# mauruszach/multimodal_diffusion

Measured on AMD Instinct MI355X. Metric: denoising steps/sec @256x256 multimodal-cond batch=32, higher is better.
Workload: dtype f32 via 3xbf16 split operands (6-term products, f32 accumulate; fp32-level error); 1 GPU; C3: 256x256 audio->video CFG denoising step (cond+null MMDiT d512 L8 H8 + noise head + DDIM), 384+37 tokens, batch 32 per GPU, DDIM 50 steps, guidance 3.5; global_batch=32, sampler_steps=50, parallelism=dp1, launch=eager, matmul=bf16x3, attn=default, cfg_halves=two HIP streams

## Files before the change

### multimodal_diffusion_amd/csrc/avd_common.h

```cpp
#pragma once
#include <hip/hip_runtime.h>
#include <stdint.h>
#include <stdio.h>
#include <stdarg.h>
#include <atomic>

#include "../../include/avdiff_hip.h"

namespace avd {

int set_error(int code, const char* fmt, ...);

#define AVD_REQUIRE(cond, code, ...)                       \
    do {                                                   \
        if (!(cond)) return avd::set_error((code), __VA_ARGS__); \
    } while (0)

#define AVD_CHECK_LAUNCH(name)                                                          \
    do {                                                                                \
        hipError_t e__ = hipGetLastError();                                             \
        if (e__ != hipSuccess)                                                          \
            return avd::set_error(AVD_ELAUNCH, "%s: %s", (name), hipGetErrorString(e__)); \
    } while (0)

struct LdsAttr {
    std::atomic<uint64_t> done{0};
    int ensure(const void* kern, int lds_bytes, const char* what);
};

static inline bool aligned16(const void* p) { return (reinterpret_cast<uintptr_t>(p) & 15u) == 0; }

typedef float f32x4 __attribute__((ext_vector_type(4)));
typedef float f32x16 __attribute__((ext_vector_type(16)));

constexpr int kWave = 64;

__device__ __forceinline__ int mfma32_row(int r, int hi) { return (r & 3) + 8 * (r >> 2) + 4 * hi; }

__device__ __forceinline__ float gelu_erf(float x) {
    const float z = x * 0.70710678118654752440f;
    const float a = fabsf(z);
    const float t = __builtin_amdgcn_rcpf(fmaf(0.3275911f, a, 1.0f));
    float p = fmaf(1.061405429f, t, -1.453152027f);
    p = fmaf(p, t, 1.421413741f);
    p = fmaf(p, t, -0.284496736f);
    p = fmaf(p, t, 0.254829592f);
    p *= t;
    const float e = __builtin_amdgcn_exp2f(-a * a * 1.4426950408889634f);
    const float er = copysignf(fmaf(-p, e, 1.0f), z);
    return 0.5f * x * (1.0f + er);
}
__device__ __forceinline__ float silu(float x) { return x / (1.0f + expf(-x)); }

template <int ACT>
__device__ __forceinline__ float apply_act(float x) {
    if constexpr (ACT == AVD_ACT_GELU) return gelu_erf(x);
    else if constexpr (ACT == AVD_ACT_SILU) return silu(x);
    else return x;
}

__device__ __forceinline__ float wave_sum(float v) {
#pragma unroll
    for (int o = 32; o > 0; o >>= 1) v += __shfl_xor(v, o, 64);
    return v;
}

struct RowMap {
    int64_t ld;
    int64_t seg;
    int64_t stride;
    __host__ __device__ __forceinline__ int64_t off(int64_t r) const {
        return seg > 0 ? (r / seg) * stride + (r % seg) * ld : r * ld;
    }
};

struct RowSegs {
    int64_t m0;
    int tok[2], samples[2];
    static RowSegs uniform(int samples, int tok) { return RowSegs{(int64_t)samples * tok, {tok, tok}, {samples, 0}}; }
    __host__ __device__ __forceinline__ int64_t rows() const { return m0 + (int64_t)samples[1] * tok[1]; }
    __host__ __device__ __forceinline__ int n_samples() const { return samples[0] + samples[1]; }
    __host__ __device__ __forceinline__ void locate(int64_t m, int& sample, int& token) const {
        const bool s1 = m >= m0;
        const unsigned r = (unsigned)(s1 ? m - m0 : m), t = (unsigned)(s1 ? tok[1] : tok[0]);
        const unsigned b = r / t;
        sample = (int)b + (s1 ? samples[0] : 0);
        token = (int)(r - b * t);
    }
    __host__ __device__ __forceinline__ int64_t row(int sample, int token) const {
        return sample < samples[0] ? (int64_t)sample * tok[0] + token : m0 + (int64_t)(sample - samples[0]) * tok[1] + token;
    }
};

struct TubeGather {
    int T, H, W, t, h, w, Ht, Wt, Nt;
    int64_t per;
    __host__ __device__ __forceinline__ int64_t row_off(int64_t row) const {
        const int64_t b = row / Nt;
        const int n = (int)(row - b * Nt);
        const int nx = n % Wt, ny = (n / Wt) % Ht, nt = n / (Wt * Ht);
        return b * per + ((int64_t)(nt * t) * H + ny * h) * W + nx * w;
    }
    __host__ __device__ __forceinline__ int64_t k_off(int k) const {
        const int dx = k % w, dy = (k / w) % h, dt = (k / (w * h)) % t, c = k / (w * h * t);
        return (((int64_t)c * T + dt) * H + dy) * W + dx;
    }
};

typedef __bf16 bf16x8 __attribute__((ext_vector_type(8)));
typedef unsigned int u32x4 __attribute__((ext_vector_type(4)));

constexpr int S3_CHUNK = 128 * 96;
constexpr int S3_PLANE = 128 * 32;

typedef __bf16 bf16x2 __attribute__((ext_vector_type(2)));
typedef float f32x2 __attribute__((ext_vector_type(2)));

__device__ __forceinline__ unsigned int pk_bf16(float a, float b) {
    const f32x2 v = {a, b};
    return __builtin_bit_cast(unsigned int, __builtin_convertvector(v, bf16x2));
}
__device__ __forceinline__ float bf16_lo(unsigned int p) { return __uint_as_float(p << 16); }
__device__ __forceinline__ float bf16_hi(unsigned int p) { return __uint_as_float(p & 0xffff0000u); }

template <bool RANGE_CHECK = true>
__device__ __forceinline__ void split8(const float* v, u32x4& H, u32x4& Mi, u32x4& Lo) {
#pragma clang fp contract(off)
    bool edge = false;
    if constexpr (RANGE_CHECK) {
        float amax = fabsf(v[0]);
#pragma unroll
        for (int e = 1; e < 8; ++e) amax = fmaxf(amax, fabsf(v[e]));
        edge = __any(amax > 3.3895313892515355e38f);
    }
#pragma unroll
    for (int e = 0; e < 4; ++e) {
        const float a = v[2 * e], b = v[2 * e + 1];
        unsigned int h = pk_bf16(a, b);
        float ra = a - bf16_lo(h), rb = b - bf16_hi(h);
        if (edge) {
            if ((h & 0x7fffu) == 0x7f80u) {
                if (fabsf(a) < __builtin_inff()) { h = (h & 0xffff8000u) | 0x7f7fu; ra = a - bf16_lo(h); } else ra = 0.f;
            }
            if ((h & 0x7fff0000u) == 0x7f800000u) {
                if (fabsf(b) < __builtin_inff()) { h = (h & 0x8000ffffu) | 0x7f7f0000u; rb = b - bf16_hi(h); } else rb = 0.f;
            }
        }
        const unsigned int m = pk_bf16(ra, rb);
        const float sa = ra - bf16_lo(m), sb = rb - bf16_hi(m);
        H[e] = h;
        Mi[e] = m;
        Lo[e] = pk_bf16(sa, sb);
    }
}

template <bool RANGE_CHECK = true>
__device__ __forceinline__ void store_split8(unsigned char* img, int64_t r, int k, int K, const float* v) {
    u32x4 H, Mi, Lo;
    split8<RANGE_CHECK>(v, H, Mi, Lo);
    const int rr = (int)(r & 127), half = (k >> 3) & 1;
    unsigned char* dst = img + ((r >> 7) * (K >> 4) + (k >> 4)) * (int64_t)S3_CHUNK + rr * 32 + ((half ^ ((rr >> 4) & 1)) << 4);
    *reinterpret_cast<u32x4*>(dst) = H;
    *reinterpret_cast<u32x4*>(dst + S3_PLANE) = Mi;
    *reinterpret_cast<u32x4*>(dst + 2 * S3_PLANE) = Lo;
}

typedef _Float16 f16x8 __attribute__((ext_vector_type(8)));
typedef _Float16 f16x2 __attribute__((ext_vector_type(2)));

__device__ __forceinline__ unsigned int pk_f16(float a, float b) {
    const f32x2 v = {a, b};
    return __builtin_bit_cast(unsigned int, __builtin_convertvector(v, f16x2));
}
__device__ __forceinline__ f32x2 unpk_f16(unsigned int p) { return __builtin_convertvector(__builtin_bit_cast(f16x2, p), f32x2); }

__device__ __forceinline__ void split8_h2(const float* v, float s, u32x4& H, u32x4& L) {
#pragma unroll
    for (int e = 0; e < 4; ++e) {
        const float a = v[2 * e] * s, b = v[2 * e + 1] * s;
        const unsigned int h = pk_f16(a, b);
        const f32x2 u = unpk_f16(h);
        H[e] = h;
        L[e] = pk_f16(a - u[0], b - u[1]);
    }
}
__device__ __forceinline__ void store_split8_h2(unsigned char* img, int64_t r, int k, int K, const float* v, float s) {
    u32x4 H, L;
    split8_h2(v, s, H, L);
    const int rr = (int)(r & 127), half = (k >> 3) & 1;
    unsigned char* dst = img + ((r >> 7) * (K >> 4) + (k >> 4)) * (int64_t)S3_CHUNK + rr * 32 + ((half ^ ((rr >> 4) & 1)) << 4);
    *reinterpret_cast<u32x4*>(dst) = H;
    *reinterpret_cast<u32x4*>(dst + S3_PLANE) = L;
}

template <bool F16>
__device__ __forceinline__ f32x16 mma16(bf16x8 a, bf16x8 b, f32x16 c) {
    if constexpr (F16)
        return __builtin_amdgcn_mfma_f32_32x32x16_f16(__builtin_bit_cast(f16x8, a), __builtin_bit_cast(f16x8, b), c, 0, 0, 0);
    else
        return __builtin_amdgcn_mfma_f32_32x32x16_bf16(a, b, c, 0, 0, 0);
}
__host__ __device__ constexpr int s3_planes(int terms) { return terms == 1 ? 1 : terms == 3 ? 2 : 3; }

constexpr int QKV3_ROWB = 384;
__host__ __device__ __forceinline__ int qkv3_npad(int n) { return (n + 63) / 64 * 64; }
__host__ __device__ __forceinline__ int qkv3_swizzle(int part, int n) {
    return part == 0 ? 0 : part == 1 ? (n >> 1) & 7 : (((n >> 1) & 1) << 2) | (((n >> 2) & 1) << 1);
}

extern bool g_prof_on;
void prof_mark(int tag, double work, hipStream_t st, bool begin);
int prof_tag_id(const char* fmt, ...);
struct ProfScope {
    int tag; hipStream_t st; bool on;
    ProfScope(int t, double work, hipStream_t s) : tag(t), st(s), on(g_prof_on) { if (on) prof_mark(tag, work, st, true); }
    ~ProfScope() { if (on) prof_mark(tag, 0.0, st, false); }
};

int gemm_f32(const float* A, RowMap am, const float* W, const float* bias, const float* R, RowMap rm,
             float* C, RowMap cm, int64_t M, int N, int K, int act, hipStream_t st);
int gemm_f32_tube(const float* z, const TubeGather& tg, const float* W, const float* bias, float* C, RowMap cm, int64_t M, int N, int K,
                  hipStream_t st);

extern int g_gemm_stages;
extern int g_gemm_force_tile;
bool gemm_f32_fold_supported(int N, int K);
int gemm_f32_fold(const float* A, RowMap am, const float* W, const float* bias, const float* R, RowMap rm, float* C, RowMap cm,
                  int64_t M, int N, int K, int act, const float* ss_in, int ss_in_cols, float sqrt_d, float eps, float* ss_out,
                  hipStream_t st);
int rowss_f32(const float* x, float* ss, int64_t rows, int d, hipStream_t st);
constexpr int kGemmSplitKMax = 4;
extern int g_gemm_splitk;
int gemm_f32_splitk_slices(int64_t M, int N, int K);
int64_t gemm_f32_splitk_ws_max_floats(int64_t M, int N, int K);
int gemm_f32_splitk(const float* A, RowMap am, const float* W, const float* bias, const float* R, RowMap rm, float* C, RowMap cm, int64_t M,
                    int N, int K, int ns, float* part, float* ss_out, hipStream_t st);

int attn_f32(const float* qkv, float* out, int B, int N, int H, int Dh, float scale, int n_query, const unsigned char* key_padding_mask,
             hipStream_t st);
int rmsnorm_f32(const float* x, RowMap xm, const float* scale, float* y, RowMap ym, int64_t rows, int d, float eps,
                hipStream_t st);
int layernorm_act_f32(const float* x, const float* gamma, const float* beta, float* y, int64_t rows, int d, float eps,
                      int act, hipStream_t st);
int weight_bounds_f32(const float* x, int64_t rows, int d, float* out2, hipStream_t st);

int64_t split3_bytes(int64_t rows, int K);
int split3_f32(const float* x, int64_t ld, void* out, int64_t rows, int K, hipStream_t st, float h2_scale = 0.f);
int split3_rows_f32(const float* x, RowMap xm, void* out, int64_t rows, int K, hipStream_t st, float h2_scale = 0.f, float* ss = nullptr);
int rmsnorm_split3_f32(const float* x, const float* scale, void* out, int64_t rows, int d, float eps, hipStream_t st, float h2_scale = 0.f);
int layernorm_act_split3_f32(const float* x, const float* gamma, const float* beta, void* out, int64_t rows, int d, float eps, int act,
                             hipStream_t st, float h2_scale = 0.f);
bool gemm_bf16x3_supported(int64_t M, int N, int K);
int attn_f32_split3(const float* qkv, void* out3, int B, int N, int H, int Dh, float scale, int n_query, hipStream_t st);
extern int g_s3_stagger;
extern int g_mlp_fused;
bool mlp_bf16x3_supported(int d, int hidden, int terms);
int mlp_bf16x3(const void* X3, const void* W1n3, const float* b1, const void* W23, const float* b2, const float* ss_in, float eps,
               const float* R, float* C, void* C3, float* ss_out, int64_t M, int d, int hidden, hipStream_t st);
extern int g_attn_m16;
extern int g_attn_pipe;
extern int g_s3_m16;
extern int g_s3_w128;
extern int g_s3_rt4;
extern int g_s3_deep4;
extern int g_s3_rt;
extern int g_vae_lat;
extern int g_vae_fold;
extern int g_codec_mfma;
extern int g_cfg_rows;
extern int g_s3_sn, g_s3_super4, g_s3_super8;
extern int g_s3_tile;
extern thread_local bool t_s3_two_streams;
int gemm_bf16x3_qkv3(const void* A3, const void* W3, const float* bias, void* img, const RowSegs& seg, int heads, int K, float qscale,
                     int terms, hipStream_t st, float ab_scale = 1.f, float c_scale = 1.f, const float* ss_in = nullptr, float eps = 0.f,
                     int64_t plan_rows = 0);
int64_t qkv3_bytes(int B, int N, int H);
int64_t attn_fp8_ws_bytes(int B, int N, int H);
int attn_fp8(const void* qkv3, void* ws, int64_t ws_bytes, float* out, void* out3, int B, int N, int H, int n_query, hipStream_t st,
             int img_terms = 6, float img_scale = 1.f, float out_scale = 1.f);
int attn_bf16x3(const void* qkv3, float* out, void* out3, int B, int N, int H, int n_query, int terms, hipStream_t st,
                float img_scale = 1.f, float out_scale = 1.f, int out_tokens = 0, const RowSegs* out_rows = nullptr);
int gemm_bf16x3(const void* A3, const void* W3, const float* bias, const float* R, float* C, void* C3, int64_t M, int N, int K,
                int act, int terms, hipStream_t st, float ab_scale = 1.f, float c_scale = 1.f, const float* ss_in = nullptr, float eps = 0.f,
                float* ss_out = nullptr, const float* gamma = nullptr, int r_seg = 0, const RowSegs* r_map = nullptr, int64_t plan_rows = 0);
bool gemm_bf16x3_resmap_supported(int terms);
bool gemm_bf16x3_rownorm_supported(int N, int terms);
extern int g_s3_splitk;
int gemm_bf16x3_splitk_slices(int64_t M, int N, int K, int terms);
int64_t gemm_bf16x3_splitk_ws_floats(int64_t M, int N, int ns);
constexpr int kS3SplitKMax = 4;
int64_t gemm_bf16x3_splitk_ws_max_floats(int64_t M, int N, int K);
int gemm_bf16x3_splitk(const void* A3, const void* W3, const float* bias, const float* R, float* C, void* C3, float* ss, int64_t M, int N,
                       int K, int terms, int ns, float* part, hipStream_t st);

}
```

### multimodal_diffusion_amd/csrc/composite.hip

```cpp
#include "avd_common.h"

#include <limits.h>
#include <stdlib.h>

#include <string.h>
#include <map>
#include <mutex>
#include <string>
#include <utility>
#include <vector>

namespace avd {

static thread_local char g_err[512] = "";

int set_error(int code, const char* fmt, ...) {
    va_list ap;
    va_start(ap, fmt);
    vsnprintf(g_err, sizeof(g_err), fmt, ap);
    va_end(ap);
    return code;
}

int LdsAttr::ensure(const void* kern, int lds_bytes, const char* what) {
    int dev = 0;
    hipError_t e = hipGetDevice(&dev);
    if (e != hipSuccess) return set_error(AVD_ELAUNCH, "%s: hipGetDevice: %s", what, hipGetErrorString(e));
    const uint64_t bit = dev < 64 ? (uint64_t)1 << dev : 0;
    if (bit && (done.load(std::memory_order_acquire) & bit)) return AVD_OK;
    e = hipFuncSetAttribute(kern, hipFuncAttributeMaxDynamicSharedMemorySize, lds_bytes);
    if (e != hipSuccess) return set_error(AVD_ELAUNCH, "%s: hipFuncSetAttribute: %s", what, hipGetErrorString(e));
    done.fetch_or(bit, std::memory_order_release);
    return AVD_OK;
}

bool g_prof_on = false;
namespace {
struct ProfRec { hipEvent_t a, b; int tag; double work; };
std::vector<ProfRec> g_recs;
std::vector<hipEvent_t> g_pool;
std::vector<std::string> g_tags;
hipEvent_t take_event() {
    if (!g_pool.empty()) { hipEvent_t e = g_pool.back(); g_pool.pop_back(); return e; }
    hipEvent_t e; (void)hipEventCreate(&e); return e;
}
}
int prof_tag_id(const char* fmt, ...) {
    char buf[160];
    va_list ap;
    va_start(ap, fmt);
    vsnprintf(buf, sizeof(buf), fmt, ap);
    va_end(ap);
    for (size_t i = 0; i < g_tags.size(); ++i)
        if (g_tags[i] == buf) return (int)i;
    g_tags.emplace_back(buf);
    return (int)g_tags.size() - 1;
}
void prof_mark(int tag, double work, hipStream_t st, bool begin) {
    if (begin) {
        ProfRec r{take_event(), take_event(), tag, work};
        (void)hipEventRecord(r.a, st);
        g_recs.push_back(r);
    } else if (!g_recs.empty()) {
        (void)hipEventRecord(g_recs.back().b, st);
    }
}

int temb_f32(const int64_t* t, const float* freqs, float* out, int B, int dim, float max_period, hipStream_t st);
int tube_patch_f32(const float* z, float* tok, int B, int C, int T, int H, int W, int t, int h, int w, hipStream_t st);
int audio_tokens_f32(const float* z, float* tok, int B, int Ca, int F, int len, int stride, hipStream_t st);
int assemble_f32(float* X2, const float* temb, const float* Xp, int B, int N, int d, int tdim, int Nt, int Np,
                 int target_first, hipStream_t st);
int assemble_rows_f32(float* X2, const int64_t* t_now, const float* freqs, const float* Xp, float* ss, int B, int N, int d, int tdim,
                      int Nt, int Np, int target_first, float max_period, hipStream_t st, const RowSegs* short_null = nullptr, int slots = 0,
                      int slot_tok = 0);
int qkv3_replicate(void* img, int img_samples, int H, int n_keys, int first_sample, int n_samples, int src, hipStream_t st);
int cfg_unpatch_ddim_f32(const float* eps2, const float* z, const int64_t* t_now, const int64_t* t_prev,
                         const float* abar, int T_train, float guidance, float eta, const float* noise, float* z_out,
                         int B, int C, int T, int H, int W, int t, int h, int w, hipStream_t st, const avd_noise_key* key = nullptr,
                         const int64_t* t_last = nullptr, float* x0_hist = nullptr, const avd_latent_guide* guide = nullptr,
                         const avd_cfg_control* ctl = nullptr, int canvas_hop = 0, int guide_hop = 0, int slots = 0,
                         const avd_apg_control* apg = nullptr, const avd_slot_key* skey = nullptr,
                         const avd_clip_guide* cguide = nullptr, const avd_slot_cfg* scfg = nullptr);
int cfg_untoken_ddim_audio_f32(const float* eps2, const float* z, const int64_t* t_now, const int64_t* t_prev,
                               const float* abar, int T_train, float guidance, float eta, const float* noise,
                               float* z_out, int B, int Ca, int F, int len, int stride, hipStream_t st,
                               const avd_noise_key* key = nullptr, const int64_t* t_last = nullptr, float* x0_hist = nullptr,
                               const avd_latent_guide* guide = nullptr, const avd_cfg_control* ctl = nullptr, int canvas_hop = 0, int guide_hop = 0,
                               int slots = 0, const avd_apg_control* apg = nullptr, const avd_slot_key* skey = nullptr,
                               const avd_clip_guide* cguide = nullptr, const avd_slot_cfg* scfg = nullptr);
int assemble_cond_f32(float* X1, const float* temb, const float* Xp, int B, int N, int d, int tdim, int Nt, int Np, int target_first,
                      hipStream_t st);
int assemble_rows_cond_f32(float* X1, const int64_t* t_now, const float* freqs, const float* Xp, float* ss, int B, int N, int d,
                           int tdim, int Nt, int Np, int target_first, float max_period, hipStream_t st);
int eps_unpatch_ddim_f32(const float* eps1, const float* z, const int64_t* t_now, const int64_t* t_prev, const float* abar, int T_train,
                         float eta, const float* noise, float* z_out, int B, int C, int T, int H, int W, int t, int h, int w,
                         hipStream_t st, const avd_noise_key* key, const int64_t* t_last, float* x0_hist, const avd_latent_guide* guide,
                         int canvas_hop = 0, int guide_hop = 0);
int eps_untoken_ddim_audio_f32(const float* eps1, const float* z, const int64_t* t_now, const int64_t* t_prev, const float* abar,
                               int T_train, float eta, const float* noise, float* z_out, int B, int Ca, int F, int len, int stride,
                               hipStream_t st, const avd_noise_key* key, const int64_t* t_last, float* x0_hist,
                               const avd_latent_guide* guide, int canvas_hop = 0, int guide_hop = 0);
int check_canvas_key(const avd_noise_key* key, int N, int64_t outer, int L, int hop, int64_t inner);
int check_slot_key(const avd_slot_key* key, int B, int64_t outer, int slot_len, int64_t inner);
int check_clip_guide(const avd_clip_guide* g, int B, int64_t outer, int L, int slots, int slot_len, int64_t inner, const float* out,
                     const float* x0_hist);
int check_canvas_guide(const avd_latent_guide* g, int N, int64_t outer, int L, int hop, int64_t inner, const float* out,
                       const float* x0_hist);
int check_latent_guide(const avd_latent_guide* g, int B, int64_t per, const float* out, const float* x0_hist);
int check_cfg_control(const avd_cfg_control* ctl, int B, int64_t per, const float* out, const float* x0_hist);
int check_apg_control(const avd_apg_control* apg, const avd_cfg_control* ctl, int B, int64_t per, const float* z, const float* out,
                      const float* x0_hist, const void* eps, int64_t eps_bytes);
int check_slot_cfg(const avd_slot_cfg* cfg, int B, int S, int64_t per_slot, int64_t per, const float* z, const float* out,
                   const float* x0_hist, const void* eps, int64_t eps_bytes);
bool overlaps(const float* a, const float* b, int64_t n);

static inline int64_t align_up(int64_t x) { return (x + 255) & ~(int64_t)255; }

struct Carver {
    char* base;
    int64_t used, cap;
    bool ok = true;
    float* take(int64_t floats) {
        float* p = reinterpret_cast<float*>(base + used);
        used += align_up(floats * (int64_t)sizeof(float));
        if (used > cap) ok = false;
        return p;
    }
};

constexpr int64_t kSplitMinRows = 6144;
constexpr int64_t kSplitMinRowsM16 = 2048;
static int g_s3_min_rows = -1;
static int g_no_fold = 0;
static int64_t split_min_rows(int terms = 3) {
    if (g_s3_min_rows >= 0) return g_s3_min_rows;
    return (terms == 0 || terms == 6) && g_s3_m16 ? kSplitMinRowsM16 : kSplitMinRows;
}
static bool core_split_capable(const avd_core_weights* w, int64_t M) {
    if (w->norm_kind != 0) return false;
    if (!gemm_bf16x3_supported(M, 3 * w->d, w->d) || !gemm_bf16x3_supported(M, w->d, w->d) ||
        !gemm_bf16x3_supported(M, w->mlp_hidden, w->d) || !gemm_bf16x3_supported(M, w->d, w->mlp_hidden))
        return false;
    for (int l = 0; l < w->n_layers; ++l) {
        const avd_block_weights& b = w->blocks[l];
        if (!b.in_proj_weight3 || !b.out_proj_weight3 || !b.fc1_weight3 || !b.fc2_weight3) return false;
    }
    return true;
}
static thread_local int64_t t_step_rows = 0;
static bool core_use_split(const avd_core_weights* w, int64_t M) {
    const int64_t Mt = t_step_rows > M ? t_step_rows : M;
    if (Mt < split_min_rows(w->split_terms) && w->split_terms != 1 && w->attn_mode != 1) return false;
    return core_split_capable(w, M);
}

static bool core_split_fold_capable(const avd_core_weights* w) {
    if (w->norm_kind != 0 || w->split_terms == 3 || w->d % 64 != 0) return false;
    for (int l = 0; l < w->n_layers; ++l)
        if (!w->blocks[l].in_proj_weight3n || !w->blocks[l].fc1_weight3n) return false;
    return true;
}
static bool core_use_split_fold(const avd_core_weights* w) { return !g_no_fold && core_split_fold_capable(w); }

static bool core_split_rownorm_capable(const avd_core_weights* w) {
    return w->norm_kind == 0 && w->split_terms == 3 && gemm_bf16x3_rownorm_supported(w->d, 3);
}
static bool core_use_split_rownorm(const avd_core_weights* w) { return !g_no_fold && core_split_rownorm_capable(w); }

static bool core_use_fold(const avd_core_weights* w) {
    if (g_no_fold || w->norm_kind != 0) return false;
    if (!gemm_f32_fold_supported(3 * w->d, w->d) || !gemm_f32_fold_supported(w->d, w->d) ||
        !gemm_f32_fold_supported(w->mlp_hidden, w->d) || !gemm_f32_fold_supported(w->d, w->mlp_hidden))
        return false;
    for (int l = 0; l < w->n_layers; ++l)
        if (!w->blocks[l].in_proj_weight_n || !w->blocks[l].fc1_weight_n) return false;
    return true;
}

#define AVD_HIP(call)                                                                        \
    do {                                                                                     \
        hipError_t e__ = (call);                                                             \
        if (e__ != hipSuccess) return set_error(AVD_ELAUNCH, "%s: %s", #call, hipGetErrorString(e__)); \
    } while (0)

static int g_core_trim = 1;
static int64_t core_trim_floats(const avd_core_weights* w, int B, int N) { return (int64_t)B * N * w->d; }
static int g_cfg_offset = 0;

static int g_cfg_dedup = 1;
[[maybe_unused]] static const bool g_cfg_dedup_env_applied = [] {
    if (const char* e = getenv("AVD_CFG_DEDUP")) g_cfg_dedup = atoll(e) != 0;
    return true;
}();

static int64_t core_split_wide_bytes(const avd_core_weights* w, int B, int N) {
    const int64_t qkv3 = qkv3_bytes(B, N, w->n_heads), fc1 = split3_bytes((int64_t)B * N, w->mlp_hidden);
    return qkv3 > fc1 ? qkv3 : fc1;
}

static int64_t core_ws_bytes(const avd_core_weights* w, int B, int N) {
    const int64_t M = (int64_t)B * N;
    const int wide = 3 * w->d > w->mlp_hidden ? 3 * w->d : w->mlp_hidden;
    int64_t fp32_path = align_up(M * w->d * 4) + align_up(M * wide * 4) + 2 * align_up(M * (w->d / 32 + 1) * 4) +
                        align_up(gemm_f32_splitk_ws_max_floats(M, w->d, w->mlp_hidden) * 4);
    if (!core_split_capable(w, M)) return fp32_path;
    const int64_t wide_b = core_split_wide_bytes(w, B, N);
    const int64_t f8_b = w->attn_mode == 1 ? attn_fp8_ws_bytes(B, N, w->n_heads) : 0;
    const int64_t fold_b = core_split_fold_capable(w) ? align_up(split3_bytes(M, w->d)) + align_up(M * (w->d / 64) * 4)
                         : core_split_rownorm_capable(w) ? align_up(split3_bytes(M, w->d)) : 0;
    const int64_t sk_b = core_split_fold_capable(w) ? align_up(gemm_bf16x3_splitk_ws_max_floats(M, w->d, w->mlp_hidden) * 4) : 0;
    const int64_t trim_b = core_split_fold_capable(w) ? align_up(core_trim_floats(w, B, N) * 4) : 0;
    const int64_t split_path = align_up(wide_b) + align_up(split3_bytes(M, w->d)) + align_up(f8_b) + fold_b + sk_b + trim_b;
    return split_path > fp32_path ? split_path : fp32_path;
}

static int check_core(const avd_core_weights* w) {
    AVD_REQUIRE(w && w->blocks && w->final_norm_scale, AVD_EINVAL, "core: null weight table");
    AVD_REQUIRE(w->d > 0 && w->n_layers > 0 && w->n_heads > 0 && w->mlp_hidden > 0, AVD_EINVAL, "core: bad dims");
    AVD_REQUIRE(w->d % w->n_heads == 0, AVD_EINVAL, "core: d_model %d not divisible by n_heads %d", w->d, w->n_heads);
    AVD_REQUIRE(w->attn_mode == 0 || w->attn_mode == 1, AVD_EINVAL, "core: attn_mode must be 0 (follow the matmul mode) or 1 (fp8)");
    AVD_REQUIRE(w->norm_kind == 0 || w->norm_kind == 1, AVD_EINVAL, "core: norm_kind must be 0 (RMSNorm) or 1 (LayerNorm)");
    AVD_REQUIRE(w->d / w->n_heads == 64, AVD_EUNSUPPORTED, "core: head_dim %d unsupported (64 only)", w->d / w->n_heads);
    AVD_REQUIRE(w->d % 4 == 0 && w->mlp_hidden % 4 == 0, AVD_EUNSUPPORTED, "core: widths must be multiples of 4");
    AVD_REQUIRE(w->split_terms == 0 || w->split_terms == 6 || w->split_terms == 9 || w->split_terms == 1 || w->split_terms == 3, AVD_EINVAL,
                "core: split_terms must be 0/6 (default), 9 (strict), 1 (plain bf16) or 3 (f16x2), got %d", w->split_terms);
    if (w->split_terms == 3) {
        for (int l = 0; l < w->n_layers; ++l)
            for (int i = 0; i < 8; ++i) {
                const float s = w->blocks[l].f16x2_scale[i];
                AVD_REQUIRE(s > 0.f && s < __builtin_inff(), AVD_EINVAL, "core: blocks[%d].f16x2_scale[%d] must be positive and finite", l, i);
            }
    }
    return AVD_OK;
}

static int core_norm(const avd_core_weights* w, const float* x, const float* scale, const float* bias, float* y, int64_t M, hipStream_t st) {
    const RowMap rd{w->d, 0, 0};
    if (w->norm_kind == 0) return rmsnorm_f32(x, rd, scale, y, rd, M, w->d, w->norm_eps, st);
    AVD_REQUIRE(bias, AVD_EINVAL, "core: norm_kind 1 (LayerNorm) needs the bias vectors");
    return layernorm_act_f32(x, scale, bias, y, M, w->d, w->norm_eps, AVD_ACT_NONE, st);
}

static bool core_dedup_ok(const avd_core_weights* w, int B2, int N, int n_out) {
    const int terms = w->split_terms;
    return B2 % 2 == 0 && n_out > 0 && n_out + 2 <= N && w->attn_mode == 0 && (terms == 0 || terms == 6 || terms == 9) && g_core_trim &&
           !g_mlp_fused && gemm_bf16x3_resmap_supported(terms) && core_use_split(w, (int64_t)B2 * N) && core_use_split_fold(w);
}

static int core_forward(const avd_core_weights* w, const float* x, float* y, int B, int N, int out_row0,
                        int n_out_rows, const unsigned char* kpm, void* ws, int64_t ws_bytes, hipStream_t st,
                        const float* ss_first = nullptr, const RowSegs* segs = nullptr, int plan_samples = 0,
                        hipEvent_t lead = nullptr, int lead_after = 0) {
    if (int rc = check_core(w)) return rc;
    AVD_REQUIRE(x && y && B > 0 && N > 0, AVD_EINVAL, "core: bad input");
    AVD_REQUIRE(out_row0 >= 0 && n_out_rows > 0 && out_row0 + n_out_rows <= N, AVD_EINVAL, "core: bad output row window");
    const int64_t M = (int64_t)B * N;
    AVD_REQUIRE(ws && ws_bytes >= core_ws_bytes(w, B, N), AVD_EWORKSPACE, "core: workspace %lld < %lld bytes",
                (long long)ws_bytes, (long long)core_ws_bytes(w, B, N));
    const int d = w->d, hid = w->mlp_hidden, H = w->n_heads;
    Carver cv{static_cast<char*>(ws), 0, ws_bytes};
    float* hbuf = cv.take(M * d);
    float* wide = cv.take(M * (3 * d > hid ? 3 * d : hid));
    const RowMap rd{d, 0, 0}, r3{3 * d, 0, 0}, rh{hid, 0, 0};
    const float scale = 1.0f / sqrtf((float)(d / H));
    const float* cur = x;
    AVD_REQUIRE(!(w->attn_mode == 1 && (kpm || w->norm_kind != 0)), AVD_EUNSUPPORTED,
                "core: attn_mode 1 (fp8 attention) cannot be combined with a key_padding_mask or norm_kind 1 (LayerNorm)");
    const int null_from = segs ? segs->samples[0] : 0;
    const int Bp = plan_samples > B ? plan_samples : B;
    AVD_REQUIRE(!segs || (null_from >= 0 && segs->samples[1] > 0 && segs->n_samples() == B && segs->tok[0] == N &&
                          segs->tok[1] == n_out_rows + 1 && segs->m0 == (int64_t)null_from * N && out_row0 == 0 && !kpm &&
                          core_dedup_ok(w, null_from ? B : Bp, N, n_out_rows)), AVD_EUNSUPPORTED,
                "core: the two-segment row layout needs the folded six-term split path with the trimmed last block");
    AVD_REQUIRE(!(w->attn_mode == 1 && !core_use_split(w, M)), AVD_EUNSUPPORTED,
                "core: attn_mode 1 (fp8 attention) reads the q|k|v image of the split-operand projections, which these weights / shapes "
                "do not take (every block needs its *_weight3 images; 3 d, d and mlp_hidden must be multiples of 256, d of 16)");
    if (!kpm && core_use_split(w, M)) {
        const int terms = w->split_terms;
        Carver cs{static_cast<char*>(ws), 0, ws_bytes};
        const int64_t wide_b = core_split_wide_bytes(w, B, N);
        float* qkv = cs.take((wide_b + 3) / 4);
        void* wide3 = qkv;
        void* hs = cs.take((split3_bytes(M, d) + 3) / 4);
        const int64_t f8_b = w->attn_mode == 1 ? attn_fp8_ws_bytes(B, N, H) : 0;
        float* f8w = cs.take((f8_b + 3) / 4);
        if (core_use_split_fold(w)) {
            void* hx = cs.take((split3_bytes(M, d) + 3) / 4);
            float* ss = cs.take(M * (d / 64));
            const int64_t Mp = (int64_t)Bp * N;
            const int ns = gemm_bf16x3_splitk_slices(Mp, d, hid, terms);
            float* part = ns ? cs.take(gemm_bf16x3_splitk_ws_floats(M, d, ns)) : nullptr;
            const bool trim = g_core_trim && out_row0 == 0 && n_out_rows < N && w->attn_mode == 0 && gemm_bf16x3_resmap_supported(terms);
            float* yc = cs.take(core_trim_floats(w, B, N));
            const bool fused = g_mlp_fused && !ns && mlp_bf16x3_supported(d, hid, terms) && gemm_bf16x3_resmap_supported(terms);
            AVD_REQUIRE(cs.ok, AVD_EWORKSPACE, "core: workspace carve %lld > %lld bytes", (long long)cs.used, (long long)cs.cap);
            const RowSegs seg = segs ? *segs : RowSegs::uniform(B, N);
            const int64_t Mr = seg.rows();
            const float qscale = scale * 1.4426950408889634f;
            auto in_proj = [&](const avd_block_weights& b) {
                if (int rc = gemm_bf16x3_qkv3(hx, b.in_proj_weight3n, b.in_proj_bias, qkv, seg, H, d, qscale, terms, st, 1.f, 1.f, ss, w->norm_eps, Mp))
                    return rc;
                return segs ? qkv3_replicate(qkv, B, H, N, null_from, B - null_from, n_out_rows, st) : (int)AVD_OK;
            };
            auto mark = [&](int l, int n) {
                if (lead && l == 0 && n == lead_after) AVD_HIP(hipEventRecord(lead, st));
                return (int)AVD_OK;
            };
            if (int rc = split3_rows_f32(cur, rd, hx, Mr, d, st, 0.f, ss)) return rc;
            for (int l = 0; l < w->n_layers; ++l) {
                const avd_block_weights& b = w->blocks[l];
                const bool last = l == w->n_layers - 1;
                const int nq = (last && out_row0 == 0) ? n_out_rows : N;
                if (last && trim) {
                    const int64_t Mc = (int64_t)B * nq, Mcp = (int64_t)Bp * nq;
                    if (int rc = in_proj(b)) return rc;
                    if (int rc = mark(l, 1)) return rc;
                    if (int rc = attn_bf16x3(qkv, nullptr, hs, B, N, H, nq, terms, st, 1.f, 1.f, nq)) return rc;
                    if (int rc = mark(l, 2)) return rc;
                    if (int rc = gemm_bf16x3(hs, b.out_proj_weight3, b.out_proj_bias, cur, yc, hx, Mc, d, d, AVD_ACT_NONE, terms, st, 1.f, 1.f,
                                             nullptr, 0.f, ss, nullptr, nq, &seg, Mcp)) return rc;
                    if (int rc = mark(l, 3)) return rc;
                    if (fused) {
                        if (int rc = mlp_bf16x3(hx, b.fc1_weight3n, b.fc1_bias, b.fc2_weight3, b.fc2_bias, ss, w->norm_eps, yc, yc, nullptr, nullptr, Mc,
                                                d, hid, st)) return rc;
                    } else {
                        if (int rc = gemm_bf16x3(hx, b.fc1_weight3n, b.fc1_bias, nullptr, nullptr, wide3, Mc, hid, d, AVD_ACT_GELU, terms, st, 1.f, 1.f,
                                                 ss, w->norm_eps, nullptr, nullptr, 0, nullptr, Mcp)) return rc;
                        if (ns) {
                            if (int rc = gemm_bf16x3_splitk(wide3, b.fc2_weight3, b.fc2_bias, yc, yc, nullptr, nullptr, Mc, d, hid, terms, ns, part,
                                                            st)) return rc;
                        } else {
                            if (int rc = gemm_bf16x3(wide3, b.fc2_weight3, b.fc2_bias, yc, yc, nullptr, Mc, d, hid, AVD_ACT_NONE, terms, st, 1.f, 1.f,
                                                     nullptr, 0.f, nullptr, nullptr, 0, nullptr, Mcp)) return rc;
                        }
                    }
                    return rmsnorm_f32(yc, rd, w->final_norm_scale, y, segs ? rd : RowMap{d, nq, (int64_t)N * d}, Mc, d, w->norm_eps, st);
                }
                if (int rc = in_proj(b)) return rc;
                if (int rc = mark(l, 1)) return rc;
                if (w->attn_mode == 1) {
                    if (int rc = attn_fp8(qkv, f8w, f8_b, nullptr, hs, B, N, H, nq, st, terms, 1.f, 1.f)) return rc;
                } else if (segs) {
                    if (int rc = attn_bf16x3(qkv, nullptr, hs, B, N, H, N, terms, st, 1.f, 1.f, 0, &seg)) return rc;
                } else {
                    if (int rc = attn_bf16x3(qkv, nullptr, hs, B, N, H, nq, terms, st, 1.f, 1.f)) return rc;
                }
                if (int rc = mark(l, 2)) return rc;
                if (int rc = gemm_bf16x3(hs, b.out_proj_weight3, b.out_proj_bias, cur, y, hx, Mr, d, d, AVD_ACT_NONE, terms, st, 1.f, 1.f, nullptr,
                                         0.f, ss, nullptr, 0, nullptr, Mp)) return rc;
                if (int rc = mark(l, 3)) return rc;
                cur = y;
                if (fused) {
                    if (int rc = mlp_bf16x3(hx, b.fc1_weight3n, b.fc1_bias, b.fc2_weight3, b.fc2_bias, ss, w->norm_eps, y, y, last ? nullptr : hx,
                                            last ? nullptr : ss, Mr, d, hid, st)) return rc;
                    continue;
                }
                if (int rc = gemm_bf16x3(hx, b.fc1_weight3n, b.fc1_bias, nullptr, nullptr, wide3, Mr, hid, d, AVD_ACT_GELU, terms, st, 1.f, 1.f, ss,
                                         w->norm_eps, nullptr, nullptr, 0, nullptr, Mp)) return rc;
                if (ns) {
                    if (int rc = gemm_bf16x3_splitk(wide3, b.fc2_weight3, b.fc2_bias, y, y, last ? nullptr : hx, last ? nullptr : ss, Mr, d, hid,
                                                    terms, ns, part, st)) return rc;
                } else if (last) {
                    if (int rc = gemm_bf16x3(wide3, b.fc2_weight3, b.fc2_bias, y, y, nullptr, Mr, d, hid, AVD_ACT_NONE, terms, st)) return rc;
                } else {
                    if (int rc = gemm_bf16x3(wide3, b.fc2_weight3, b.fc2_bias, y, y, hx, Mr, d, hid, AVD_ACT_NONE, terms, st, 1.f, 1.f, nullptr, 0.f,
                                             ss, nullptr, 0, nullptr, Mp)) return rc;
                }
            }
            return rmsnorm_f32(y, rd, w->final_norm_scale, y, rd, Mr, d, w->norm_eps, st);
        }
        const bool rown = core_use_split_rownorm(w);
        void* hn = rown ? cs.take((split3_bytes(M, d) + 3) / 4) : hs;
        AVD_REQUIRE(cs.ok, AVD_EWORKSPACE, "core: workspace carve %lld > %lld bytes", (long long)cs.used, (long long)cs.cap);
        for (int l = 0; l < w->n_layers; ++l) {
            const avd_block_weights& b = w->blocks[l];
            const bool last = l == w->n_layers - 1;
            const int nq = (last && out_row0 == 0) ? n_out_rows : N;
            const bool h2 = terms == 3;
            const float* fs = b.f16x2_scale;
            const float s_n1 = h2 ? fs[4] : 0.f, s_qkv = h2 ? fs[5] : 1.f, s_n2 = h2 ? fs[6] : 0.f, s_fc1 = h2 ? fs[7] : 1.f;
            const float w_in = h2 ? fs[0] : 1.f, w_out = h2 ? fs[1] : 1.f, w_fc1 = h2 ? fs[2] : 1.f, w_fc2 = h2 ? fs[3] : 1.f;
            if (!rown || l == 0)
                if (int rc = rmsnorm_split3_f32(cur, b.norm1_scale, hn, M, d, w->norm_eps, st, s_n1)) return rc;
            if (int rc = gemm_bf16x3_qkv3(hn, b.in_proj_weight3, b.in_proj_bias, qkv, RowSegs::uniform(B, N), H, d, scale * 1.4426950408889634f, terms, st,
                                          h2 ? s_n1 * w_in : 1.f, s_qkv)) return rc;
            if (w->attn_mode == 1) {
                if (int rc = attn_fp8(qkv, f8w, f8_b, nullptr, hs, B, N, H, nq, st, terms, s_qkv, s_qkv)) return rc;
            } else {
                if (int rc = attn_bf16x3(qkv, nullptr, hs, B, N, H, nq, terms, st, s_qkv, s_qkv)) return rc;
            }
            if (rown) {
                if (int rc = gemm_bf16x3(hs, b.out_proj_weight3, b.out_proj_bias, cur, y, hn, M, d, d, AVD_ACT_NONE, terms, st, s_qkv * w_out, s_n2,
                                         nullptr, w->norm_eps, nullptr, b.norm2_scale)) return rc;
                cur = y;
            } else {
                if (int rc = gemm_bf16x3(hs, b.out_proj_weight3, b.out_proj_bias, cur, y, nullptr, M, d, d, AVD_ACT_NONE, terms, st,
                                         h2 ? s_qkv * w_out : 1.f, 1.f)) return rc;
                cur = y;
                if (int rc = rmsnorm_split3_f32(y, b.norm2_scale, hn, M, d, w->norm_eps, st, s_n2)) return rc;
            }
            if (int rc = gemm_bf16x3(hn, b.fc1_weight3, b.fc1_bias, nullptr, nullptr, wide3, M, hid, d, AVD_ACT_GELU, terms, st,
                                     h2 ? s_n2 * w_fc1 : 1.f, s_fc1)) return rc;
            if (rown && !last) {
                const avd_block_weights& nb = w->blocks[l + 1];
                if (int rc = gemm_bf16x3(wide3, b.fc2_weight3, b.fc2_bias, y, y, hn, M, d, hid, AVD_ACT_NONE, terms, st, s_fc1 * w_fc2,
                                         nb.f16x2_scale[4], nullptr, w->norm_eps, nullptr, nb.norm1_scale)) return rc;
            } else {
                if (int rc = gemm_bf16x3(wide3, b.fc2_weight3, b.fc2_bias, y, y, nullptr, M, d, hid, AVD_ACT_NONE, terms, st,
                                         h2 ? s_fc1 * w_fc2 : 1.f, 1.f)) return rc;
            }
        }
        return rmsnorm_f32(y, rd, w->final_norm_scale, y, rd, M, d, w->norm_eps, st);
    }
    if (core_use_fold(w)) {
        float* ssA = cv.take(M * (d / 32 + 1));
        float* ssB = cv.take(M * (d / 32 + 1));
        const int nsf = gemm_f32_splitk_slices(M, d, hid);
        float* partf = nsf ? cv.take((int64_t)nsf * M * d) : nullptr;
        AVD_REQUIRE(cv.ok, AVD_EWORKSPACE, "core: workspace carve %lld > %lld bytes", (long long)cv.used, (long long)cv.cap);
        const float sqrt_d = (float)sqrt((double)d);
        const float* ssA_in = ss_first;
        if (!ssA_in) {
            if (int rc = rowss_f32(cur, ssA, M, d, st)) return rc;
            ssA_in = ssA;
        }
        int colsA = 1;
        for (int l = 0; l < w->n_layers; ++l) {
            const avd_block_weights& b = w->blocks[l];
            const bool last = l == w->n_layers - 1;
            const int nq = (last && out_row0 == 0) ? n_out_rows : N;
            if (int rc = gemm_f32_fold(cur, rd, b.in_proj_weight_n, b.in_proj_bias, nullptr, rd, wide, r3, M, 3 * d, d, AVD_ACT_NONE,
                                       l == 0 ? ssA_in : ssA, colsA, sqrt_d, w->norm_eps, nullptr, st)) return rc;
            if (int rc = attn_f32(wide, hbuf, B, N, H, d / H, scale, nq, kpm, st)) return rc;
            if (int rc = gemm_f32_fold(hbuf, rd, b.out_proj_weight, b.out_proj_bias, cur, rd, y, rd, M, d, d, AVD_ACT_NONE, nullptr, 0,
                                       1.f, 0.f, ssB, st)) return rc;
            cur = y;
            if (int rc = gemm_f32_fold(y, rd, b.fc1_weight_n, b.fc1_bias, nullptr, rd, wide, rh, M, hid, d, AVD_ACT_GELU, ssB, d / 32,
                                       sqrt_d, w->norm_eps, nullptr, st)) return rc;
            if (nsf) {
                if (int rc = gemm_f32_splitk(wide, rh, b.fc2_weight, b.fc2_bias, y, rd, y, rd, M, d, hid, nsf, partf, ssA, st)) return rc;
            } else {
                if (int rc = gemm_f32_fold(wide, rh, b.fc2_weight, b.fc2_bias, y, rd, y, rd, M, d, hid, AVD_ACT_NONE, nullptr, 0, 1.f, 0.f,
                                           ssA, st)) return rc;
            }
            colsA = d / 32;
        }
        return rmsnorm_f32(y, rd, w->final_norm_scale, y, rd, M, d, w->norm_eps, st);
    }
    for (int l = 0; l < w->n_layers; ++l) {
        const avd_block_weights& b = w->blocks[l];
        const bool last = l == w->n_layers - 1;
        const int nq = (last && out_row0 == 0) ? n_out_rows : N;
        if (int rc = core_norm(w, cur, b.norm1_scale, b.norm1_bias, hbuf, M, st)) return rc;
        if (int rc = gemm_f32(hbuf, rd, b.in_proj_weight, b.in_proj_bias, nullptr, rd, wide, r3, M, 3 * d, d, AVD_ACT_NONE, st)) return rc;
        if (int rc = attn_f32(wide, hbuf, B, N, H, d / H, scale, nq, kpm, st)) return rc;
        if (int rc = gemm_f32(hbuf, rd, b.out_proj_weight, b.out_proj_bias, cur, rd, y, rd, M, d, d, AVD_ACT_NONE, st)) return rc;
        cur = y;
        if (int rc = core_norm(w, y, b.norm2_scale, b.norm2_bias, hbuf, M, st)) return rc;
        if (int rc = gemm_f32(hbuf, rd, b.fc1_weight, b.fc1_bias, nullptr, rd, wide, rh, M, hid, d, AVD_ACT_GELU, st)) return rc;
        if (int rc = gemm_f32(wide, rh, b.fc2_weight, b.fc2_bias, y, rd, y, rd, M, d, hid, AVD_ACT_NONE, st)) return rc;
    }
    return core_norm(w, y, w->final_norm_scale, w->final_norm_bias, y, M, st);
}

static bool head_split_capable(const avd_head_weights* w, int64_t rows) {
    if (w->split_terms == 0) return false;
    if (!w->input_proj_weight3 || !w->out_proj_weight3 || (w->n_shared > 0 && !w->shared_lin_weight3)) return false;
    for (int j = 0; j < w->n_shared; ++j)
        if (!w->shared_lin_weight3[j]) return false;
    if (w->split_terms == 3 && !w->f16x2_scale) return false;
    return gemm_bf16x3_supported(rows, w->hidden, w->d_in) && gemm_bf16x3_supported(rows, w->hidden, w->hidden) &&
           gemm_bf16x3_supported(rows, w->d_out, w->hidden);
}
static thread_local int64_t t_step_head_rows = 0;
static bool head_use_split(const avd_head_weights* w, int64_t rows) {
    return (t_step_head_rows > rows ? t_step_head_rows : rows) >= split_min_rows() && head_split_capable(w, rows);
}

static int64_t head_ws_bytes(const avd_head_weights* w, int64_t rows) {
    const int64_t fp32_path = 2 * align_up(rows * w->hidden * 4);
    if (!head_split_capable(w, rows)) return fp32_path;
    const int wide = w->d_in > w->hidden ? w->d_in : w->hidden;
    const int64_t split_path = 2 * align_up(split3_bytes(rows, wide)) + align_up(rows * w->hidden * 4);
    return split_path > fp32_path ? split_path : fp32_path;
}

static int head_forward(const avd_head_weights* w, const float* h, RowMap hm, int64_t rows, float* out, void* ws,
                        int64_t ws_bytes, hipStream_t st, int64_t plan_rows = 0) {
    AVD_REQUIRE(w && h && out, AVD_EINVAL, "head: null pointer");
    AVD_REQUIRE(w->d_in > 0 && w->hidden > 0 && w->d_out > 0 && w->n_shared >= 0, AVD_EINVAL, "head: bad dims");
    AVD_REQUIRE(w->input_proj_weight && w->out_proj_weight, AVD_EINVAL, "head: null weights");
    AVD_REQUIRE(w->n_shared == 0 || (w->shared_lin_weight && w->shared_lin_bias && w->shared_ln_weight && w->shared_ln_bias),
                AVD_EINVAL, "head: null shared-trunk tables");
    AVD_REQUIRE(w->split_terms == 0 || w->split_terms == 6 || w->split_terms == 9 || w->split_terms == 1 || w->split_terms == 3, AVD_EINVAL,
                "head: split_terms must be 0 (fp32), 6, 9, 1 or 3, got %d", w->split_terms);
    AVD_REQUIRE(ws && ws_bytes >= head_ws_bytes(w, rows), AVD_EWORKSPACE, "head: workspace too small");
    Carver cv{static_cast<char*>(ws), 0, ws_bytes};
    const RowMap rh{w->hidden, 0, 0}, ro{w->d_out, 0, 0};
    if (head_use_split(w, rows)) {
        const int terms = w->split_terms, n = w->n_shared;
        const bool h2 = terms == 3;
        const float* fs = w->f16x2_scale;
        if (h2)
            for (int i = 0; i < 2 * (n + 2); ++i)
                AVD_REQUIRE(fs[i] > 0.f && fs[i] < __builtin_inff(), AVD_EINVAL, "head: f16x2_scale[%d] must be positive and finite", i);
        auto wsc = [&](int i) { return h2 ? fs[i] : 1.f; };
        auto asc = [&](int i) { return h2 ? fs[n + 2 + i] : 0.f; };
        const int wide = w->d_in > w->hidden ? w->d_in : w->hidden;
        void* imgA = cv.take((split3_bytes(rows, wide) + 3) / 4);
        void* imgB = cv.take((split3_bytes(rows, wide) + 3) / 4);
        float* t2 = cv.take(rows * w->hidden);
        if (int rc = split3_rows_f32(h, hm, imgA, rows, w->d_in, st, asc(0))) return rc;
        if (int rc = gemm_bf16x3(imgA, w->input_proj_weight3, w->input_proj_bias, nullptr, nullptr, imgB, rows, w->hidden, w->d_in, AVD_ACT_NONE,
                                 terms, st, h2 ? asc(0) * wsc(0) : 1.f, h2 ? asc(1) : 1.f, nullptr, 0.f, nullptr, nullptr, 0, nullptr, plan_rows)) return rc;
        void* cur = imgB;
        void* nxt = imgA;
        for (int j = 0; j < n; ++j) {
            if (int rc = gemm_bf16x3(cur, w->shared_lin_weight3[j], w->shared_lin_bias[j], nullptr, t2, nullptr, rows, w->hidden, w->hidden,
                                     AVD_ACT_NONE, terms, st, h2 ? asc(1 + j) * wsc(1 + j) : 1.f, 1.f, nullptr, 0.f, nullptr, nullptr, 0, nullptr, plan_rows)) return rc;
            if (int rc = layernorm_act_split3_f32(t2, w->shared_ln_weight[j], w->shared_ln_bias[j], nxt, rows, w->hidden, w->ln_eps, w->act, st,
                                                  asc(2 + j))) return rc;
            void* t = cur; cur = nxt; nxt = t;
        }
        return gemm_bf16x3(cur, w->out_proj_weight3, w->out_proj_bias, nullptr, out, nullptr, rows, w->d_out, w->hidden, AVD_ACT_NONE, terms, st,
                           h2 ? asc(1 + n) * wsc(1 + n) : 1.f, 1.f, nullptr, 0.f, nullptr, nullptr, 0, nullptr, plan_rows);
    }
    float* t1 = cv.take(rows * w->hidden);
    float* t2 = cv.take(rows * w->hidden);
    if (int rc = gemm_f32(h, hm, w->input_proj_weight, w->input_proj_bias, nullptr, rh, t1, rh, rows, w->hidden, w->d_in, AVD_ACT_NONE, st)) return rc;
    for (int j = 0; j < w->n_shared; ++j) {
        if (int rc = gemm_f32(t1, rh, w->shared_lin_weight[j], w->shared_lin_bias[j], nullptr, rh, t2, rh, rows, w->hidden, w->hidden, AVD_ACT_NONE, st)) return rc;
        if (int rc = layernorm_act_f32(t2, w->shared_ln_weight[j], w->shared_ln_bias[j], t1, rows, w->hidden, w->ln_eps, w->act, st)) return rc;
    }
    return gemm_f32(t1, rh, w->out_proj_weight, w->out_proj_bias, nullptr, ro, out, ro, rows, w->d_out, w->hidden, AVD_ACT_NONE, st);
}

static int check_embed(const avd_embed_desc* e) {
    AVD_REQUIRE(e, AVD_EINVAL, "embed: null descriptor");
    AVD_REQUIRE(e->B > 0 && e->d > 0 && e->tdim >= 0, AVD_EINVAL, "embed: bad widths");
    AVD_REQUIRE(e->temb_add ? e->tdim == e->d : e->tdim < e->d, AVD_EINVAL,
                "embed: timestep width %d does not fit token width %d in %s mode", e->tdim, e->d, e->temb_add ? "add" : "concat");
    AVD_REQUIRE(e->d % 4 == 0 && e->tdim % 4 == 0, AVD_EUNSUPPORTED, "embed: d and tdim must be multiples of 4");
    AVD_REQUIRE(e->Nt > 0 && e->Np >= 0, AVD_EINVAL, "embed: bad token counts");
    if (e->target_kind == 0) {
        AVD_REQUIRE(e->p0 > 0 && e->p1 > 0 && e->p2 > 0 && e->T % e->p0 == 0 && e->H % e->p1 == 0 && e->W % e->p2 == 0,
                    AVD_EINVAL, "tube sizes must divide latent dims");
        AVD_REQUIRE(e->Nt == (e->T / e->p0) * (e->H / e->p1) * (e->W / e->p2), AVD_EINVAL, "embed: token count mismatch");
    } else if (e->target_kind == 1) {
        AVD_REQUIRE(e->p0 > 0 && e->p1 > 0 && e->T >= e->p0, AVD_EINVAL, "embed: bad audio chunking");
        AVD_REQUIRE(e->Nt == (e->T - e->p0) / e->p1 + 1, AVD_EINVAL, "embed: token count mismatch");
    } else {
        return set_error(AVD_EINVAL, "embed: unknown target_kind %d", e->target_kind);
    }
    return AVD_OK;
}
static int embed_tok_dim(const avd_embed_desc* e) {
    return e->target_kind == 0 ? e->C * e->p0 * e->p1 * e->p2 : e->C * e->p0;
}
static int64_t embed_ws_floats(const avd_embed_desc* e) {
    return align_up((int64_t)e->B * e->Nt * embed_tok_dim(e) * 4) / 4 + align_up((int64_t)e->B * (e->tdim > 0 ? e->tdim : 1) * 4) / 4;
}

static int embed_slots(const avd_embed_desc* e, int& S, int& tok) {
    if (e->target_kind == 0) {
        S = e->T / e->p0;
        tok = (e->H / e->p1) * (e->W / e->p2);
    } else {
        AVD_REQUIRE(e->p1 == e->p0, AVD_EUNSUPPORTED, "slot timesteps need non-overlapping audio chunks (stride %d == len %d)", e->p1, e->p0);
        S = e->Nt;
        tok = 1;
    }
    return AVD_OK;
}

static int embed_cfg_pair(const avd_embed_desc* e, const float* z, const float* Wt, const float* bt,
                          const int64_t* t_now, const float* Xp, float* tok_ws, float* X2, hipStream_t st, float* ss_out = nullptr,
                          bool cond_only = false, const RowSegs* short_null = nullptr, int slots = 0) {
    if (int rc = check_embed(e)) return rc;
    int slot_tok = 0;
    if (slots) {
        int S = 0;
        if (int rc = embed_slots(e, S, slot_tok)) return rc;
        AVD_REQUIRE(slots == S, AVD_EINVAL, "embed: slots %d must equal the geometry's %d slots along the sliding axis", slots, S);
        AVD_REQUIRE(!e->temb_add && !cond_only, AVD_EINVAL, "embed: slot timesteps take the concat embedding of the CFG pair (temb_add == 0)");
    }
    AVD_REQUIRE(z && Wt && t_now && tok_ws && X2 && (e->Np == 0 || Xp), AVD_EINVAL, "embed: null pointer");
    AVD_REQUIRE(!short_null || (!cond_only && !e->temb_add && e->target_first && e->Np >= 1), AVD_EINVAL,
                "embed: the short null half is the concat-mode CFG pair with the target rows first");
    const int B = e->B, d = e->d, N = e->Nt + e->Np, D = embed_tok_dim(e);
    float* tok = tok_ws;
    float* temb = tok_ws + align_up((int64_t)B * e->Nt * D * 4) / 4;
    const bool fuse_patch = e->target_kind == 0 && !e->temb_add && e->p2 % 4 == 0 && e->W % 4 == 0 && D % 4 == 0 && aligned16(z);
    if (e->target_kind == 0) {
        if (!fuse_patch)
            if (int rc = tube_patch_f32(z, tok, B, e->C, e->T, e->H, e->W, e->p0, e->p1, e->p2, st)) return rc;
    } else {
        if (int rc = audio_tokens_f32(z, tok, B, e->C, e->T, e->p0, e->p1, st)) return rc;
    }
    if (e->tdim > 0 && e->temb_add)
        if (int rc = temb_f32(t_now, e->temb_freqs, temb, B, e->tdim, 10000.f, st)) return rc;
    float* c0 = X2 + (e->target_first ? 0 : (int64_t)e->Np * d);
    const RowMap cm{d, e->Nt, (int64_t)N * d};
    if (e->temb_add) {
        const RowMap rm{0, e->Nt, (int64_t)e->tdim};
        if (int rc = gemm_f32(tok, RowMap{D, 0, 0}, Wt, bt, temb, rm, c0, cm, (int64_t)B * e->Nt, d, D, AVD_ACT_NONE, st)) return rc;
        if (cond_only) return assemble_cond_f32(X2, temb, Xp, B, N, d, 0, e->Nt, e->Np, e->target_first, st);
        return assemble_f32(X2, temb, Xp, B, N, d, 0, e->Nt, e->Np, e->target_first, st);
    }
    if (fuse_patch) {
        const TubeGather tg{e->T, e->H, e->W, e->p0, e->p1, e->p2, e->H / e->p1, e->W / e->p2, e->Nt, (int64_t)e->C * e->T * e->H * e->W};
        if (int rc = gemm_f32_tube(z, tg, Wt, bt, c0, cm, (int64_t)B * e->Nt, d - e->tdim, D, st)) return rc;
    } else {
        if (int rc = gemm_f32(tok, RowMap{D, 0, 0}, Wt, bt, nullptr, cm, c0, cm, (int64_t)B * e->Nt, d - e->tdim, D, AVD_ACT_NONE, st)) return rc;
    }
    if (cond_only)
        return assemble_rows_cond_f32(X2, t_now, e->temb_freqs, Xp, ss_out, B, N, d, e->tdim, e->Nt, e->Np, e->target_first, 10000.f, st);
    return assemble_rows_f32(X2, t_now, e->temb_freqs, Xp, ss_out, B, N, d, e->tdim, e->Nt, e->Np, e->target_first, 10000.f, st,
                             short_null, slots, slot_tok);
}

struct AuxState { hipStream_t aux = nullptr; hipEvent_t fork = nullptr, join = nullptr, lead = nullptr; };
static std::mutex g_aux_mu;
static std::map<std::pair<int, hipStream_t>, AuxState> g_aux_map;
static int ensure_aux(hipStream_t st, AuxState& out) {
    int dev = 0;
    AVD_HIP(hipGetDevice(&dev));
    std::lock_guard<std::mutex> lk(g_aux_mu);
    AuxState& a = g_aux_map[{dev, st}];
    if (!a.aux) {
        AVD_HIP(hipStreamCreateWithFlags(&a.aux, hipStreamNonBlocking));
        AVD_HIP(hipEventCreateWithFlags(&a.fork, hipEventDisableTiming));
        AVD_HIP(hipEventCreateWithFlags(&a.join, hipEventDisableTiming));
        AVD_HIP(hipEventCreateWithFlags(&a.lead, hipEventDisableTiming));
    }
    out = a;
    return AVD_OK;
}

struct StepPlan {
    int64_t x2, tok, core, head, eps, ss, total;
    int N, D;
    int64_t rows;
};
static int plan_step(const avd_step_desc* s, StepPlan& p) {
    AVD_REQUIRE(s && s->core && s->head, AVD_EINVAL, "step: null descriptor");
    if (int rc = check_embed(&s->embed)) return rc;
    if (int rc = check_core(s->core)) return rc;
    const avd_embed_desc& e = s->embed;
    AVD_REQUIRE(e.d == s->core->d && s->head->d_in == e.d, AVD_EINVAL, "step: width mismatch between embed/core/head");
    p.N = e.Nt + e.Np;
    p.D = embed_tok_dim(&e);
    AVD_REQUIRE(s->head->d_out == p.D, AVD_EINVAL, "step: head d_out %d != token dim %d", s->head->d_out, p.D);
    p.rows = (int64_t)2 * e.B * e.Nt;
    p.x2 = align_up((int64_t)2 * e.B * p.N * e.d * 4);
    p.tok = align_up(embed_ws_floats(&e) * 4);
    const int64_t halves = 2 * core_ws_bytes(s->core, e.B, p.N), whole = core_ws_bytes(s->core, 2 * e.B, p.N);
    p.core = halves > whole ? halves : whole;
    const int64_t head_halves = 2 * head_ws_bytes(s->head, p.rows / 2), head_whole = head_ws_bytes(s->head, p.rows);
    p.head = head_halves > head_whole ? head_halves : head_whole;
    p.eps = align_up(p.rows * p.D * 4);
    p.ss = align_up((int64_t)2 * e.B * p.N * 4);
    p.total = p.x2 + p.tok + p.core + p.head + p.ss + p.eps;
    return AVD_OK;
}

struct StepWs {
    StepPlan p;
    float *X, *tok;
    void *core_ws, *head_ws;
    float *ssx, *eps;
};
static int open_step(const avd_step_desc* s, const float* z, const float* z_out, const int64_t* t_now, const int64_t* t_prev,
                     void* workspace, int64_t workspace_bytes, StepWs& ws) {
    StepPlan& p = ws.p;
    if (int rc = plan_step(s, p)) return rc;
    AVD_REQUIRE(z && z_out && t_now && t_prev && s->alpha_bar && s->adapt_w, AVD_EINVAL, "step: null pointer");
    AVD_REQUIRE(z != z_out, AVD_EINVAL, "step: z_out must not alias z");
    AVD_REQUIRE(workspace && workspace_bytes >= p.total, AVD_EWORKSPACE, "step: workspace %lld < %lld bytes",
                (long long)workspace_bytes, (long long)p.total);
    char* w = static_cast<char*>(workspace);
    ws.X = reinterpret_cast<float*>(w);
    ws.tok = reinterpret_cast<float*>(w + p.x2);
    ws.core_ws = w + p.x2 + p.tok;
    ws.head_ws = w + p.x2 + p.tok + p.core;
    ws.ssx = reinterpret_cast<float*>(w + p.x2 + p.tok + p.core + p.head);
    ws.eps = reinterpret_cast<float*>(w + p.x2 + p.tok + p.core + p.head + p.ss);
    return AVD_OK;
}

}

using namespace avd;

extern "C" int avd_abi_version(void) { return AVD_ABI_VERSION; }
extern "C" const char* avd_last_error(void) { return g_err; }

constexpr int kNoExcept = INT_MIN;
struct TuneKey { const char* key; const char* env; int* var; int lo, hi; bool boolean; int except = kNoExcept; };
static const TuneKey kTuneKeys[] = {
    {"s3_tile", "AVD_S3_TILE", &g_s3_tile, INT_MIN, INT_MAX, false},
    {"s3_m16", "AVD_S3_M16", &g_s3_m16, INT_MIN, INT_MAX, false},
    {"s3_rt", "AVD_S3_RT", &g_s3_rt, INT_MIN, INT_MAX, false},
    {"s3_rt4", "AVD_S3_RT4", &g_s3_rt4, 0, 8, false, 1},
    {"s3_deep4", "AVD_S3_DEEP4", &g_s3_deep4, INT_MIN, INT_MAX, true},
    {"s3_w128", "AVD_S3_W128", &g_s3_w128, INT_MIN, INT_MAX, false},
    {"s3_splitk", "AVD_S3_SPLITK", &g_s3_splitk, 0, kS3SplitKMax, false},
    {"s3_stagger", "AVD_S3_STAGGER", &g_s3_stagger, INT_MIN, INT_MAX, false},
    {"cfg_rows", "AVD_CFG_ROWS", &g_cfg_rows, INT_MIN, INT_MAX, true},
    {"vae_lat", "AVD_VAE_LAT", &g_vae_lat, INT_MIN, INT_MAX, true},
    {"vae_fold", "AVD_VAE_FOLD", &g_vae_fold, INT_MIN, INT_MAX, true},
    {"codec_mfma", "AVD_CODEC_MFMA", &g_codec_mfma, INT_MIN, INT_MAX, true},
    {"s3_sn", "AVD_S3_SN", &g_s3_sn, INT_MIN, INT_MAX, false},
    {"s3_super4", "AVD_S3_SUPER4", &g_s3_super4, INT_MIN, INT_MAX, false},
    {"s3_super8", "AVD_S3_SUPER8", &g_s3_super8, INT_MIN, INT_MAX, false},
    {"attn_pipe", "AVD_ATTN_PIPE", &g_attn_pipe, INT_MIN, INT_MAX, false},
    {"attn_m16", "AVD_ATTN_M16", &g_attn_m16, INT_MIN, INT_MAX, false},
    {"core_trim", "AVD_CORE_TRIM", &g_core_trim, INT_MIN, INT_MAX, true},
    {"cfg_offset", "AVD_CFG_OFFSET", &g_cfg_offset, 0, 3, false},
    {"mlp_fused", "AVD_MLP_FUSED", &g_mlp_fused, INT_MIN, INT_MAX, false},
    {"gemm_tile", "AVD_GEMM_TILE", &g_gemm_force_tile, INT_MIN, INT_MAX, false},
    {"gemm_stages", "AVD_GEMM_STAGES", &g_gemm_stages, INT_MIN, INT_MAX, false},
    {"gemm_splitk", "AVD_GEMM_SPLITK", &g_gemm_splitk, 0, kGemmSplitKMax, false},
    {"s3_min_rows", "AVD_S3_MIN_ROWS", &g_s3_min_rows, INT_MIN, INT_MAX, false},
    {"no_fold", "AVD_NO_FOLD", &g_no_fold, INT_MIN, INT_MAX, true},
};
static void tune_store(const TuneKey& t, int64_t value) { *t.var = t.boolean ? value != 0 : (int)value; }
[[maybe_unused]] static const bool g_tune_env_applied = [] {
    for (const TuneKey& t : kTuneKeys)
        if (const char* e = getenv(t.env)) {
            const long long v = atoll(e);
            tune_store(t, v < t.lo ? t.lo : v > t.hi ? t.hi : v);
        }
    return true;
}();

extern "C" int avd_tune_set(const char* key, int64_t value) {
    AVD_REQUIRE(key, AVD_EINVAL, "tune_set: null key");
    for (const TuneKey& t : kTuneKeys) {
        if (strcmp(key, t.key)) continue;
        AVD_REQUIRE(value >= t.lo && value <= t.hi && value != t.except, AVD_EINVAL, "tune_set: %s does not take %lld", key, (long long)value);
        tune_store(t, value);
        return AVD_OK;
    }
    return set_error(AVD_EINVAL, "tune_set: unknown key '%s'", key);
}

extern "C" int avd_cfg_dedup_set(int on) {
    const int prev = g_cfg_dedup;
    g_cfg_dedup = on != 0;
    return prev;
}

extern "C" int avd_device_arch(char* buf, int buflen) {
    AVD_REQUIRE(buf && buflen > 0, AVD_EINVAL, "device_arch: bad buffer");
    hipDeviceProp_t prop;
    int dev = 0;
    hipError_t e = hipGetDevice(&dev);
    if (e != hipSuccess) return set_error(AVD_ELAUNCH, "hipGetDevice: %s", hipGetErrorString(e));
    e = hipGetDeviceProperties(&prop, dev);
    if (e != hipSuccess) return set_error(AVD_ELAUNCH, "hipGetDeviceProperties: %s", hipGetErrorString(e));
    strncpy(buf, prop.gcnArchName, buflen - 1);
    buf[buflen - 1] = 0;
    return AVD_OK;
}

extern "C" int64_t avd_core_workspace_bytes(const avd_core_weights* w, int B, int N) {
    if (!w || B <= 0 || N <= 0) return -1;
    return core_ws_bytes(w, B, N);
}
extern "C" int avd_core_forward_f32(const avd_core_weights* w, const float* x, float* y, int B, int N, int out_row0,
                                    int n_out_rows, const uint8_t* key_padding_mask, void* workspace, int64_t workspace_bytes,
                                    avd_stream_t stream) {
    return core_forward(w, x, y, B, N, out_row0, n_out_rows, key_padding_mask, workspace, workspace_bytes,
                        static_cast<hipStream_t>(stream));
}

extern "C" int64_t avd_head_workspace_bytes(const avd_head_weights* w, int64_t rows) {
    if (!w || rows < 0) return -1;
    return head_ws_bytes(w, rows);
}
extern "C" int avd_head_forward_f32(const avd_head_weights* w, const float* h, int64_t ldh, int64_t seg_rows,
                                    int64_t seg_stride, int64_t rows, float* out, void* workspace,
                                    int64_t workspace_bytes, avd_stream_t stream) {
    return head_forward(w, h, RowMap{ldh, seg_rows, seg_stride}, rows, out, workspace, workspace_bytes,
                        static_cast<hipStream_t>(stream));
}

extern "C" int64_t avd_embed_workspace_floats(const avd_embed_desc* e) {
    if (check_embed(e)) return -1;
    return embed_ws_floats(e);
}
extern "C" int avd_embed_cfg_pair_f32(const avd_embed_desc* desc, const float* z_target, const float* Wt,
                                      const float* bt, const int64_t* t_now, const float* Xp, float* tok_ws, float* X2,
                                      avd_stream_t stream) {
    return embed_cfg_pair(desc, z_target, Wt, bt, t_now, Xp, tok_ws, X2, static_cast<hipStream_t>(stream));
}

extern "C" int avd_embed_cfg_pair_slots_f32(const avd_embed_desc* desc, const float* z_target, const float* Wt, const float* bt,
                                            const int64_t* t_now, int slots, const float* Xp, float* tok_ws, float* X2,
                                            avd_stream_t stream) {
    AVD_REQUIRE(slots > 0, AVD_EINVAL, "embed_cfg_pair_slots: slots must be > 0 (got %d)", slots);
    return embed_cfg_pair(desc, z_target, Wt, bt, t_now, Xp, tok_ws, X2, static_cast<hipStream_t>(stream), nullptr, false, nullptr, slots);
}

extern "C" int avd_embed_cond_f32(const avd_embed_desc* desc, const float* z_target, const float* Wt, const float* bt,
                                  const int64_t* t_now, const float* Xp, float* tok_ws, float* X1, float* ss, avd_stream_t stream) {
    return embed_cfg_pair(desc, z_target, Wt, bt, t_now, Xp, tok_ws, X1, static_cast<hipStream_t>(stream), ss, true);
}

extern "C" int64_t avd_step_workspace_bytes(const avd_step_desc* s) {
    StepPlan p;
    if (plan_step(s, p)) return -1;
    return p.total;
}

static int denoise_step(const avd_step_desc* s, const avd_noise_key* key, const float* z, const float* Xp, const int64_t* t_now,
                        const int64_t* t_prev, const float* noise, float* z_out, void* workspace, int64_t workspace_bytes,
                        avd_stream_t stream, const int64_t* t_last = nullptr, float* x0_hist = nullptr,
                        const avd_latent_guide* guide = nullptr, const avd_cfg_control* ctl = nullptr, int canvas_hop = 0,
                        int guide_hop = 0, int slots = 0, const avd_apg_control* apg = nullptr, const avd_slot_key* skey = nullptr,
                        const avd_clip_guide* cguide = nullptr, const avd_slot_cfg* scfg = nullptr) {
    StepWs ws;
    if (int rc = open_step(s, z, z_out, t_now, t_prev, workspace, workspace_bytes, ws)) return rc;
    auto& [p, X2, tok, core_ws, head_ws, ssx, eps2] = ws;
    hipStream_t st = static_cast<hipStream_t>(stream);
    const avd_embed_desc& e = s->embed;
    const bool have_ss = !e.temb_add;

    const bool dedup = g_cfg_dedup && (!s->split_streams || s->split_streams == 2) && !e.temb_add && e.target_first && e.Np >= 2 &&
                       core_dedup_ok(s->core, 2 * e.B, p.N, e.Nt);
    const bool two = s->split_streams == 2 ? dedup : s->split_streams != 0;
    const RowSegs seg{(int64_t)e.B * p.N, {p.N, e.Nt + 1}, {e.B, e.B}};
    if (int rc = embed_cfg_pair(&e, z, s->adapt_w, s->adapt_b, t_now, Xp, tok, X2, st, ssx, false, dedup ? &seg : nullptr, slots)) return rc;
    const int row0 = e.target_first ? 0 : e.Np;
    const RowMap hm{e.d, e.Nt, (int64_t)p.N * e.d};
    if (dedup && !two) {
        if (int rc = core_forward(s->core, X2, X2, 2 * e.B, p.N, 0, e.Nt, nullptr, core_ws, p.core, st, nullptr, &seg)) return rc;
        if (int rc = head_forward(s->head, X2, RowMap{e.d, 0, 0}, p.rows, eps2, head_ws, p.head, st)) return rc;
    } else if (!two) {
        if (int rc = core_forward(s->core, X2, X2, 2 * e.B, p.N, row0, e.Nt, nullptr, core_ws, p.core, st, have_ss ? ssx : nullptr)) return rc;
        if (int rc = head_forward(s->head, X2 + (int64_t)row0 * e.d, hm, p.rows, eps2, head_ws, p.head, st)) return rc;
    } else {
        AuxState ax;
        if (int rc = ensure_aux(st, ax)) return rc;
        hipStream_t g_aux = ax.aux;
        hipEvent_t g_fork = ax.fork, g_join = ax.join;
        const int64_t half_rows = (int64_t)e.B * p.N * e.d;
        const int64_t hc = p.core / 2, hh = p.head / 2;
        AVD_HIP(hipEventRecord(g_fork, st));
        AVD_HIP(hipStreamWaitEvent(g_aux, g_fork, 0));
        struct TwoStreams {
            TwoStreams(int64_t rows, int64_t head_rows) { t_s3_two_streams = true; t_step_rows = rows; t_step_head_rows = head_rows; }
            ~TwoStreams() { t_s3_two_streams = false; t_step_rows = 0; t_step_head_rows = 0; }
        } two_streams_scope((int64_t)2 * e.B * p.N, p.rows);
        if (dedup) {
            const RowSegs null_seg{0, {p.N, e.Nt + 1}, {0, e.B}};
            float* xn = X2 + seg.m0 * e.d;
            float* eps_n = eps2 + (p.rows / 2) * p.D;
            if (int rc = core_forward(s->core, X2, X2, e.B, p.N, 0, e.Nt, nullptr, core_ws, hc, st, nullptr, nullptr, 2 * e.B,
                                      g_cfg_offset ? ax.lead : nullptr, g_cfg_offset)) return rc;
            if (int rc = head_forward(s->head, X2, hm, p.rows / 2, eps2, head_ws, hh, st, p.rows)) return rc;
            if (g_cfg_offset) AVD_HIP(hipStreamWaitEvent(g_aux, ax.lead, 0));
            if (int rc = core_forward(s->core, xn, xn, e.B, p.N, 0, e.Nt, nullptr, static_cast<char*>(core_ws) + hc, hc, g_aux, nullptr,
                                      &null_seg, 2 * e.B)) return rc;
            if (int rc = head_forward(s->head, xn, RowMap{e.d, 0, 0}, p.rows / 2, eps_n, static_cast<char*>(head_ws) + hh, hh,
                                      g_aux, p.rows)) return rc;
        }
        for (int half = 0; half < 2 && !dedup; ++half) {
            hipStream_t hs = half ? g_aux : st;
            float* xh = X2 + half * half_rows;
            if (int rc = core_forward(s->core, xh, xh, e.B, p.N, row0, e.Nt, nullptr, static_cast<char*>(core_ws) + half * hc, hc, hs,
                                      have_ss ? ssx + (int64_t)half * e.B * p.N : nullptr)) return rc;
            if (int rc = head_forward(s->head, xh + (int64_t)row0 * e.d, hm, p.rows / 2, eps2 + half * (p.rows / 2) * p.D,
                                      static_cast<char*>(head_ws) + half * hh, hh, hs)) return rc;
        }
        AVD_HIP(hipEventRecord(g_join, g_aux));
        AVD_HIP(hipStreamWaitEvent(st, g_join, 0));
    }
    if (e.target_kind == 0)
        return cfg_unpatch_ddim_f32(eps2, z, t_now, t_prev, s->alpha_bar, s->T_train, s->guidance, s->eta, noise, z_out,
                                    e.B, e.C, e.T, e.H, e.W, e.p0, e.p1, e.p2, st, key, t_last, x0_hist, guide, ctl, canvas_hop,
                                    guide_hop, slots, apg, skey, cguide, scfg);
    return cfg_untoken_ddim_audio_f32(eps2, z, t_now, t_prev, s->alpha_bar, s->T_train, s->guidance, s->eta, noise, z_out,
                                      e.B, e.C, e.T, e.p0, e.p1, st, key, t_last, x0_hist, guide, ctl, canvas_hop, guide_hop, slots, apg,
                                      skey, cguide, scfg);
}

static int denoise_step_cond(const avd_step_desc* s, const avd_noise_key* key, const float* z, const float* Xp, const int64_t* t_now,
                             const int64_t* t_prev, const float* noise, float* z_out, void* workspace, int64_t workspace_bytes,
                             avd_stream_t stream, const int64_t* t_last, float* x0_hist, const avd_latent_guide* guide,
                             int canvas_hop = 0, int guide_hop = 0) {
    StepWs ws;
    if (int rc = open_step(s, z, z_out, t_now, t_prev, workspace, workspace_bytes, ws)) return rc;
    auto& [p, X1, tok, core_ws, head_ws, ssx, eps1] = ws;
    hipStream_t st = static_cast<hipStream_t>(stream);
    const avd_embed_desc& e = s->embed;
    const bool have_ss = !e.temb_add;

    if (int rc = embed_cfg_pair(&e, z, s->adapt_w, s->adapt_b, t_now, Xp, tok, X1, st, ssx, true)) return rc;
    const int row0 = e.target_first ? 0 : e.Np;
    const RowMap hm{e.d, e.Nt, (int64_t)p.N * e.d};
    if (int rc = core_forward(s->core, X1, X1, e.B, p.N, row0, e.Nt, nullptr, core_ws, p.core / 2, st, have_ss ? ssx : nullptr)) return rc;
    if (int rc = head_forward(s->head, X1 + (int64_t)row0 * e.d, hm, p.rows / 2, eps1, head_ws, p.head / 2, st)) return rc;
    if (e.target_kind == 0)
        return eps_unpatch_ddim_f32(eps1, z, t_now, t_prev, s->alpha_bar, s->T_train, s->eta, noise, z_out, e.B, e.C, e.T, e.H, e.W, e.p0,
                                    e.p1, e.p2, st, key, t_last, x0_hist, guide, canvas_hop, guide_hop);
    return eps_untoken_ddim_audio_f32(eps1, z, t_now, t_prev, s->alpha_bar, s->T_train, s->eta, noise, z_out, e.B, e.C, e.T, e.p0, e.p1, st,
                                      key, t_last, x0_hist, guide, canvas_hop, guide_hop);
}

enum { NEED_KEY = 1, NEED_HIST = 2, NEED_GUIDE = 4, NEED_CTL = 8, TAKES_SDE = 16 };
static int check_step_options(const char* what, int need, const avd_step_desc* s, const avd_noise_key* key, const int64_t* t_last,
                              const float* x0_hist, const float* z, const float* z_out, const avd_latent_guide* g,
                              const avd_cfg_control* ctl, const float* noise, bool takes_noise = false) {
    AVD_REQUIRE(s, AVD_EINVAL, "step: null descriptor");
    const int B = s->embed.B;
    const int64_t n = (int64_t)B * s->embed.C * s->embed.T * s->embed.H * s->embed.W, per = B > 0 ? n / B : 0;
    if (ctl || (need & NEED_CTL))
        if (int rc = check_cfg_control(ctl, B, per, z_out, x0_hist)) return rc;
    if (g || (need & NEED_GUIDE))
        if (int rc = check_latent_guide(g, B, per, z_out, x0_hist)) return rc;
    AVD_REQUIRE(!(need & NEED_HIST) || (t_last && x0_hist), AVD_EINVAL, "%s: null t_last or x0_hist", what);
    AVD_REQUIRE(!t_last == !x0_hist, AVD_EINVAL, "%s: t_last and x0_hist go together (the DPM-Solver++(2M) update)", what);
    if (x0_hist) {
        AVD_REQUIRE(s->eta == 0.f || (need & TAKES_SDE), AVD_EINVAL,
                    "%s: DPM-Solver++(2M) needs eta == 0 here (eta > 0 is avd_denoise_step_dpmpp_2m_sde_f32)", what);
        AVD_REQUIRE(!(z && overlaps(x0_hist, z, n)) && !(z_out && overlaps(x0_hist, z_out, n)), AVD_EINVAL,
                    "%s: x0_hist must not alias z or z_out", what);
    }
    AVD_REQUIRE(key || !(need & NEED_KEY), AVD_EINVAL, "%s: null noise key", what);
    AVD_REQUIRE(!(noise && key), AVD_EINVAL, "%s: pass a noise tensor or a noise key, not both", what);
    AVD_REQUIRE(!(noise && g), AVD_EINVAL, "%s: unseeded noise is not supported with a latent guide (pass a noise key)", what);
    AVD_REQUIRE(s->eta == 0.f || key || noise, AVD_EINVAL, "%s: eta > 0 needs a noise key%s", what,
                takes_noise && !g ? " or a noise tensor" : " (unseeded noise is not supported here)");
    if (key)
        AVD_REQUIRE(key->sample_offset >= 0 && key->sample_offset + (int64_t)B <= ((int64_t)1 << 32), AVD_EINVAL,
                    "%s: sample_offset %lld + B %d must lie in [0, 2^32]", what, (long long)key->sample_offset, B);
    return AVD_OK;
}

extern "C" int avd_denoise_step_cond_f32(const avd_step_desc* s, const avd_latent_guide* g, const avd_noise_key* key,
                                         const int64_t* t_last, float* x0_hist, const float* z, const float* Xp, const int64_t* t_now,
                                         const int64_t* t_prev, const float* noise, float* z_out, void* workspace,
                                         int64_t workspace_bytes, avd_stream_t stream) {
    if (int rc = check_step_options("denoise_step_cond", 0, s, key, t_last, x0_hist, z, z_out, g, nullptr, noise, true)) return rc;
    return denoise_step_cond(s, key, z, Xp, t_now, t_prev, noise, z_out, workspace, workspace_bytes, stream, t_last, x0_hist, g);
}

extern "C" int avd_denoise_step_f32(const avd_step_desc* s, const float* z, const float* Xp, const int64_t* t_now,
                                    const int64_t* t_prev, const float* noise, float* z_out, void* workspace,
                                    int64_t workspace_bytes, avd_stream_t stream) {
    return denoise_step(s, nullptr, z, Xp, t_now, t_prev, noise, z_out, workspace, workspace_bytes, stream);
}

extern "C" int avd_denoise_step_slots_f32(const avd_step_desc* s, const float* z, const float* Xp, const int64_t* t_now,
                                          const int64_t* t_prev, int slots, float* z_out, void* workspace, int64_t workspace_bytes,
                                          avd_stream_t stream) {
    AVD_REQUIRE(s, AVD_EINVAL, "denoise_step_slots: null descriptor");
    AVD_REQUIRE(s->eta == 0.f, AVD_EINVAL, "denoise_step_slots: slot timesteps take the DDIM update at eta == 0 (eta is %g)", (double)s->eta);
    AVD_REQUIRE(!s->embed.temb_add, AVD_EINVAL, "denoise_step_slots: slot timesteps take the concat embedding (temb_add == 0)");
    if (int rc = check_embed(&s->embed)) return rc;
    int S = 0, tok = 0;
    if (int rc = embed_slots(&s->embed, S, tok)) return rc;
    AVD_REQUIRE(slots == S, AVD_EINVAL, "denoise_step_slots: slots %d must equal the geometry's %d slots along the sliding axis", slots, S);
    return denoise_step(s, nullptr, z, Xp, t_now, t_prev, nullptr, z_out, workspace, workspace_bytes, stream, nullptr, nullptr, nullptr,
                        nullptr, 0, 0, slots);
}

extern "C" int avd_denoise_step_slots_dpmpp_2m_f32(const avd_step_desc* s, const float* z, const float* Xp, const int64_t* t_last,
                                                   const int64_t* t_now, const int64_t* t_prev, int slots, float* x0_hist, float* z_out,
                                                   void* workspace, int64_t workspace_bytes, avd_stream_t stream) {
    AVD_REQUIRE(s, AVD_EINVAL, "denoise_step_slots_dpmpp_2m: null descriptor");
    AVD_REQUIRE(s->eta == 0.f, AVD_EINVAL, "denoise_step_slots_dpmpp_2m: slot timesteps take the ODE update at eta == 0 (eta is %g)",
                (double)s->eta);
    AVD_REQUIRE(!s->embed.temb_add, AVD_EINVAL, "denoise_step_slots_dpmpp_2m: slot timesteps take the concat embedding (temb_add == 0)");
    if (int rc = check_embed(&s->embed)) return rc;
    int S = 0, tok = 0;
    if (int rc = embed_slots(&s->embed, S, tok)) return rc;
    AVD_REQUIRE(slots == S, AVD_EINVAL, "denoise_step_slots_dpmpp_2m: slots %d must equal the geometry's %d slots along the sliding axis",
                slots, S);
    if (int rc = check_step_options("denoise_step_slots_dpmpp_2m", NEED_HIST, s, nullptr, t_last, x0_hist, z, z_out, nullptr, nullptr, nullptr))
        return rc;
    AVD_REQUIRE(aligned16(x0_hist), AVD_EUNSUPPORTED, "denoise_step_slots_dpmpp_2m: x0_hist must be 16-byte aligned");
    return denoise_step(s, nullptr, z, Xp, t_now, t_prev, nullptr, z_out, workspace, workspace_bytes, stream, t_last, x0_hist, nullptr,
                        nullptr, 0, 0, slots);
}

extern "C" int avd_denoise_step_slots_seeded_f32(const avd_step_desc* s, const avd_slot_key* key, const int64_t* t_last, float* x0_hist,
                                                 const float* z, const float* Xp, const int64_t* t_now, const int64_t* t_prev, int slots,
                                                 float* z_out, void* workspace, int64_t workspace_bytes, avd_stream_t stream) {
    AVD_REQUIRE(s, AVD_EINVAL, "denoise_step_slots_seeded: null descriptor");
    AVD_REQUIRE(key, AVD_EINVAL, "denoise_step_slots_seeded: null slot key");
    AVD_REQUIRE(!s->embed.temb_add, AVD_EINVAL, "denoise_step_slots_seeded: slot timesteps take the concat embedding (temb_add == 0)");
    if (int rc = check_embed(&s->embed)) return rc;
    int S = 0, tok = 0;
    if (int rc = embed_slots(&s->embed, S, tok)) return rc;
    AVD_REQUIRE(slots == S, AVD_EINVAL, "denoise_step_slots_seeded: slots %d must equal the geometry's %d slots along the sliding axis", slots,
                S);
    const avd_embed_desc& e = s->embed;
    AVD_REQUIRE(!t_last == !x0_hist, AVD_EINVAL, "denoise_step_slots_seeded: t_last and x0_hist go together (the DPM-Solver++(2M) update)");
    if (x0_hist) {
        const int64_t n = (int64_t)e.B * e.C * e.T * e.H * e.W;
        AVD_REQUIRE(!(z && overlaps(x0_hist, z, n)) && !(z_out && overlaps(x0_hist, z_out, n)), AVD_EINVAL,
                    "denoise_step_slots_seeded: x0_hist must not alias z or z_out");
        AVD_REQUIRE(aligned16(x0_hist), AVD_EUNSUPPORTED, "denoise_step_slots_seeded: x0_hist must be 16-byte aligned");
    }
    if (s->eta > 0.f)
        if (int rc = check_slot_key(key, e.B, e.C, e.p0, (int64_t)e.H * e.W)) return rc;
    return denoise_step(s, nullptr, z, Xp, t_now, t_prev, nullptr, z_out, workspace, workspace_bytes, stream, t_last, x0_hist, nullptr,
                        nullptr, 0, 0, slots, nullptr, key);
}

extern "C" int avd_denoise_step_slots_guided_f32(const avd_step_desc* s, const avd_slot_key* key, const avd_clip_guide* guide,
                                                 const int64_t* t_last, float* x0_hist, const float* z, const float* Xp,
                                                 const int64_t* t_now, const int64_t* t_prev, int slots, float* z_out, void* workspace,
                                                 int64_t workspace_bytes, avd_stream_t stream) {
    AVD_REQUIRE(s, AVD_EINVAL, "denoise_step_slots_guided: null descriptor");
    AVD_REQUIRE(guide, AVD_EINVAL, "denoise_step_slots_guided: null clip guide");
    AVD_REQUIRE(key || !(s->eta > 0.f), AVD_EINVAL, "denoise_step_slots_guided: eta > 0 needs a slot key");
    AVD_REQUIRE(!s->embed.temb_add, AVD_EINVAL, "denoise_step_slots_guided: slot timesteps take the concat embedding (temb_add == 0)");
    if (int rc = check_embed(&s->embed)) return rc;
    int S = 0, tok = 0;
    if (int rc = embed_slots(&s->embed, S, tok)) return rc;
    AVD_REQUIRE(slots == S, AVD_EINVAL, "denoise_step_slots_guided: slots %d must equal the geometry's %d slots along the sliding axis", slots,
                S);
    const avd_embed_desc& e = s->embed;
    AVD_REQUIRE(!t_last == !x0_hist, AVD_EINVAL, "denoise_step_slots_guided: t_last and x0_hist go together (the DPM-Solver++(2M) update)");
    if (x0_hist) {
        const int64_t n = (int64_t)e.B * e.C * e.T * e.H * e.W;
        AVD_REQUIRE(!(z && overlaps(x0_hist, z, n)) && !(z_out && overlaps(x0_hist, z_out, n)), AVD_EINVAL,
                    "denoise_step_slots_guided: x0_hist must not alias z or z_out");
        AVD_REQUIRE(aligned16(x0_hist), AVD_EUNSUPPORTED, "denoise_step_slots_guided: x0_hist must be 16-byte aligned");
    }
    if (int rc = check_clip_guide(guide, e.B, e.C, e.T, S, e.p0, (int64_t)e.H * e.W, z_out, x0_hist)) return rc;
    if (s->eta > 0.f) {
        if (int rc = check_slot_key(key, e.B, e.C, e.p0, (int64_t)e.H * e.W)) return rc;
        AVD_REQUIRE(key->first == guide->first && key->stride == guide->stride && key->cursor == guide->cursor, AVD_EINVAL,
                    "denoise_step_slots_guided: the slot key's first / stride / cursor must equal the clip guide's");
    }
    return denoise_step(s, nullptr, z, Xp, t_now, t_prev, nullptr, z_out, workspace, workspace_bytes, stream, t_last, x0_hist, nullptr,
                        nullptr, 0, 0, slots, nullptr, s->eta > 0.f ? key : nullptr, guide);
}

extern "C" int avd_denoise_step_slots_cfg_f32(const avd_step_desc* s, const avd_slot_cfg* cfg, const avd_slot_key* key,
                                              const avd_clip_guide* guide, const int64_t* t_last, float* x0_hist, const float* z,
                                              const float* Xp, const int64_t* t_now, const int64_t* t_prev, int slots, float* z_out,
                                              void* workspace, int64_t workspace_bytes, avd_stream_t stream) {
    AVD_REQUIRE(s, AVD_EINVAL, "denoise_step_slots_cfg: null descriptor");
    AVD_REQUIRE(cfg, AVD_EINVAL, "denoise_step_slots_cfg: null slot CFG control");
    AVD_REQUIRE(key || !(s->eta > 0.f), AVD_EINVAL, "denoise_step_slots_cfg: eta > 0 needs a slot key");
    AVD_REQUIRE(!s->embed.temb_add, AVD_EINVAL, "denoise_step_slots_cfg: slot timesteps take the concat embedding (temb_add == 0)");
    if (int rc = check_embed(&s->embed)) return rc;
    int S = 0, tok = 0;
    if (int rc = embed_slots(&s->embed, S, tok)) return rc;
    AVD_REQUIRE(slots == S, AVD_EINVAL, "denoise_step_slots_cfg: slots %d must equal the geometry's %d slots along the sliding axis", slots, S);
    const avd_embed_desc& e = s->embed;
    const int64_t per = (int64_t)e.C * e.T * e.H * e.W;
    const int64_t per_slot = e.target_kind == 0 ? (int64_t)e.C * e.p0 * e.H * e.W : (int64_t)e.C * e.p0;
    if (int rc = check_slot_cfg(cfg, e.B, S, per_slot, per, z, z_out, x0_hist, workspace, workspace_bytes)) return rc;
    AVD_REQUIRE(!t_last == !x0_hist, AVD_EINVAL, "denoise_step_slots_cfg: t_last and x0_hist go together (the DPM-Solver++(2M) update)");
    if (x0_hist) {
        AVD_REQUIRE(!(z && overlaps(x0_hist, z, e.B * per)) && !(z_out && overlaps(x0_hist, z_out, e.B * per)), AVD_EINVAL,
                    "denoise_step_slots_cfg: x0_hist must not alias z or z_out");
        AVD_REQUIRE(aligned16(x0_hist), AVD_EUNSUPPORTED, "denoise_step_slots_cfg: x0_hist must be 16-byte aligned");
    }
    if (guide)
        if (int rc = check_clip_guide(guide, e.B, e.C, e.T, S, e.p0, (int64_t)e.H * e.W, z_out, x0_hist)) return rc;
    if (s->eta > 0.f) {
        if (int rc = check_slot_key(key, e.B, e.C, e.p0, (int64_t)e.H * e.W)) return rc;
        AVD_REQUIRE(!guide || (key->first == guide->first && key->stride == guide->stride && key->cursor == guide->cursor), AVD_EINVAL,
                    "denoise_step_slots_cfg: the slot key's first / stride / cursor must equal the clip guide's");
    }
    return denoise_step(s, nullptr, z, Xp, t_now, t_prev, nullptr, z_out, workspace, workspace_bytes, stream, t_last, x0_hist, nullptr,
                        nullptr, 0, 0, slots, nullptr, s->eta > 0.f ? key : nullptr, guide, cfg);
}

extern "C" int avd_denoise_step_seeded_f32(const avd_step_desc* s, const avd_noise_key* key, const float* z, const float* Xp,
                                           const int64_t* t_now, const int64_t* t_prev, float* z_out, void* workspace,
                                           int64_t workspace_bytes, avd_stream_t stream) {
    if (int rc = check_step_options("denoise_step_seeded", NEED_KEY, s, key, nullptr, nullptr, z, z_out, nullptr, nullptr, nullptr)) return rc;
    return denoise_step(s, key, z, Xp, t_now, t_prev, nullptr, z_out, workspace, workspace_bytes, stream);
}

extern "C" int avd_denoise_step_dpmpp_2m_f32(const avd_step_desc* s, const float* z, const float* Xp, const int64_t* t_last,
                                             const int64_t* t_now, const int64_t* t_prev, float* x0_hist, float* z_out, void* workspace,
                                             int64_t workspace_bytes, avd_stream_t stream) {
    if (int rc = check_step_options("denoise_step_dpmpp_2m", NEED_HIST, s, nullptr, t_last, x0_hist, z, z_out, nullptr, nullptr, nullptr))
        return rc;
    return denoise_step(s, nullptr, z, Xp, t_now, t_prev, nullptr, z_out, workspace, workspace_bytes, stream, t_last, x0_hist);
}

extern "C" int avd_denoise_step_guided_f32(const avd_step_desc* s, const avd_latent_guide* g, const avd_noise_key* key,
                                           const int64_t* t_last, float* x0_hist, const float* z, const float* Xp, const int64_t* t_now,
                                           const int64_t* t_prev, float* z_out, void* workspace, int64_t workspace_bytes,
                                           avd_stream_t stream) {
    if (int rc = check_step_options("denoise_step_guided", NEED_GUIDE, s, key, t_last, x0_hist, z, z_out, g, nullptr, nullptr)) return rc;
    return denoise_step(s, key, z, Xp, t_now, t_prev, nullptr, z_out, workspace, workspace_bytes, stream, t_last, x0_hist, g);
}

extern "C" int avd_denoise_step_cfg_f32(const avd_step_desc* s, const avd_cfg_control* ctl, const avd_latent_guide* g,
                                        const avd_noise_key* key, const int64_t* t_last, float* x0_hist, const float* z, const float* Xp,
                                        const int64_t* t_now, const int64_t* t_prev, float* z_out, void* workspace,
                                        int64_t workspace_bytes, avd_stream_t stream) {
    if (int rc = check_step_options("denoise_step_cfg", NEED_CTL, s, key, t_last, x0_hist, z, z_out, g, ctl, nullptr)) return rc;
    return denoise_step(s, key, z, Xp, t_now, t_prev, nullptr, z_out, workspace, workspace_bytes, stream, t_last, x0_hist, g, ctl);
}

extern "C" int avd_denoise_step_canvas_f32(const avd_step_desc* s, const avd_noise_key* key, int hop, const avd_cfg_control* ctl,
                                           const avd_latent_guide* g, int cond_only, const float* z, const float* Xp,
                                           const int64_t* t_now, const int64_t* t_prev, float* z_out, void* workspace,
                                           int64_t workspace_bytes, avd_stream_t stream) {
    AVD_REQUIRE(s, AVD_EINVAL, "denoise_step_canvas: null descriptor");
    AVD_REQUIRE(key, AVD_EINVAL, "denoise_step_canvas: null noise key");
    AVD_REQUIRE(s->eta > 0.f, AVD_EINVAL, "denoise_step_canvas: canvas keying is the seeded eta > 0 DDIM step (eta is %g)", (double)s->eta);
    AVD_REQUIRE(!(cond_only && ctl), AVD_EINVAL, "denoise_step_canvas: a cond-only step takes no CFG control");
    const avd_embed_desc& e = s->embed;
    if (int rc = check_canvas_key(key, e.B, e.C, e.T, hop, (int64_t)e.H * e.W)) return rc;
    if (int rc = check_step_options("denoise_step_canvas", NEED_KEY, s, key, nullptr, nullptr, z, z_out, g, ctl, nullptr)) return rc;
    if (cond_only)
        return denoise_step_cond(s, key, z, Xp, t_now, t_prev, nullptr, z_out, workspace, workspace_bytes, stream, nullptr, nullptr, g, hop);
    return denoise_step(s, key, z, Xp, t_now, t_prev, nullptr, z_out, workspace, workspace_bytes, stream, nullptr, nullptr, g, ctl, hop);
}

extern "C" int avd_denoise_step_dpmpp_2m_sde_f32(const avd_step_desc* s, const avd_noise_key* key, int canvas_hop,
                                                 const avd_cfg_control* ctl, const avd_latent_guide* g, int cond_only,
                                                 const int64_t* t_last, float* x0_hist, const float* z, const float* Xp,
                                                 const int64_t* t_now, const int64_t* t_prev, float* z_out, void* workspace,
                                                 int64_t workspace_bytes, avd_stream_t stream) {
    AVD_REQUIRE(s, AVD_EINVAL, "denoise_step_dpmpp_2m_sde: null descriptor");
    AVD_REQUIRE(s->eta > 0.f, AVD_EINVAL, "denoise_step_dpmpp_2m_sde: the SDE form needs eta > 0 (eta is %g: avd_denoise_step_dpmpp_2m_f32)",
                (double)s->eta);
    AVD_REQUIRE(key, AVD_EINVAL, "denoise_step_dpmpp_2m_sde: null noise key (the SDE form draws seeded noise only)");
    AVD_REQUIRE(t_last && x0_hist, AVD_EINVAL, "denoise_step_dpmpp_2m_sde: null t_last or x0_hist");
    AVD_REQUIRE(!(cond_only && ctl), AVD_EINVAL, "denoise_step_dpmpp_2m_sde: a cond-only step takes no CFG control");
    AVD_REQUIRE(canvas_hop >= 0, AVD_EINVAL, "denoise_step_dpmpp_2m_sde: canvas_hop must be >= 0 (0: per-sample keying), got %d", canvas_hop);
    const avd_embed_desc& e = s->embed;
    if (canvas_hop)
        if (int rc = check_canvas_key(key, e.B, e.C, e.T, canvas_hop, (int64_t)e.H * e.W)) return rc;
    if (int rc = check_step_options("denoise_step_dpmpp_2m_sde", NEED_KEY | NEED_HIST | TAKES_SDE, s, key, t_last, x0_hist, z, z_out, g, ctl,
                                    nullptr)) return rc;
    if (cond_only)
        return denoise_step_cond(s, key, z, Xp, t_now, t_prev, nullptr, z_out, workspace, workspace_bytes, stream, t_last, x0_hist, g,
                                 canvas_hop);
    return denoise_step(s, key, z, Xp, t_now, t_prev, nullptr, z_out, workspace, workspace_bytes, stream, t_last, x0_hist, g, ctl, canvas_hop);
}

extern "C" int avd_denoise_step_canvas_guided_f32(const avd_step_desc* s, const avd_latent_guide* g, int hop, const avd_noise_key* key,
                                                  const avd_cfg_control* ctl, int cond_only, const int64_t* t_last, float* x0_hist,
                                                  const float* z, const float* Xp, const int64_t* t_now, const int64_t* t_prev,
                                                  float* z_out, void* workspace, int64_t workspace_bytes, avd_stream_t stream) {
    AVD_REQUIRE(s, AVD_EINVAL, "denoise_step_canvas_guided: null descriptor");
    AVD_REQUIRE(g, AVD_EINVAL, "denoise_step_canvas_guided: null latent guide");
    AVD_REQUIRE(!(cond_only && ctl), AVD_EINVAL, "denoise_step_canvas_guided: a cond-only step takes no CFG control");
    AVD_REQUIRE(s->eta >= 0.f, AVD_EINVAL, "denoise_step_canvas_guided: eta must be >= 0");
    const bool noisy = s->eta > 0.f;
    AVD_REQUIRE(!noisy || key, AVD_EINVAL,
                "denoise_step_canvas_guided: eta > 0 under a canvas-keyed guide needs a noise key (the step's noise is canvas-keyed with "
                "the guide's hop; per-sample or unseeded noise is refused)");
    const avd_embed_desc& e = s->embed;
    if (int rc = check_canvas_guide(g, e.B, e.C, e.T, hop, (int64_t)e.H * e.W, z_out, x0_hist)) return rc;
    if (noisy)
        if (int rc = check_canvas_key(key, e.B, e.C, e.T, hop, (int64_t)e.H * e.W)) return rc;
    const avd_noise_key* k = noisy ? key : nullptr;
    if (int rc = check_step_options("denoise_step_canvas_guided", NEED_GUIDE | TAKES_SDE, s, k, t_last, x0_hist, z, z_out, g, ctl, nullptr))
        return rc;
    if (cond_only)
        return denoise_step_cond(s, k, z, Xp, t_now, t_prev, nullptr, z_out, workspace, workspace_bytes, stream, t_last, x0_hist, g,
                                 noisy ? hop : 0, hop);
    return denoise_step(s, k, z, Xp, t_now, t_prev, nullptr, z_out, workspace, workspace_bytes, stream, t_last, x0_hist, g, ctl,
// ... 60 lines not shown
```

### multimodal_diffusion_amd/csrc/rowops.hip

```cpp
#include "avd_common.h"

namespace avd {

constexpr int ROW_MAXV = 8;

template <int NV>
__global__ __launch_bounds__(256) void rmsnorm_kernel(const float* x, RowMap xm,
                                                      const float* __restrict__ scale, float* y,
                                                      RowMap ym, int64_t rows, int d, float eps, float sqrt_d) {
    const int lane = threadIdx.x & 63;
    const int64_t row = (int64_t)blockIdx.x * 4 + (threadIdx.x >> 6);
    if (row >= rows) return;
    const float* xr = x + xm.off(row);
    f32x4 v[NV];
    float ss = 0.f;
#pragma unroll
    for (int i = 0; i < NV; ++i) {
        const int c = (lane + 64 * i) * 4;
        if (c < d) {
            v[i] = *reinterpret_cast<const f32x4*>(xr + c);
            ss += v[i][0] * v[i][0] + v[i][1] * v[i][1] + v[i][2] * v[i][2] + v[i][3] * v[i][3];
        }
    }
    ss = wave_sum(ss);
    const float den = sqrtf(ss) / sqrt_d + eps;
    float* yr = y + ym.off(row);
#pragma unroll
    for (int i = 0; i < NV; ++i) {
        const int c = (lane + 64 * i) * 4;
        if (c < d) {
            const f32x4 s = *reinterpret_cast<const f32x4*>(scale + c);
            f32x4 o = {s[0] * v[i][0] / den, s[1] * v[i][1] / den, s[2] * v[i][2] / den, s[3] * v[i][3] / den};
            *reinterpret_cast<f32x4*>(yr + c) = o;
        }
    }
}

template <int NV>
__global__ __launch_bounds__(256) void layernorm_act_kernel(const float* x,
                                                            const float* __restrict__ gamma,
                                                            const float* __restrict__ beta, float* y,
                                                            int64_t rows, int d, float eps, int act) {
    const int lane = threadIdx.x & 63;
    const int64_t row = (int64_t)blockIdx.x * 4 + (threadIdx.x >> 6);
    if (row >= rows) return;
    const float* xr = x + row * d;
    f32x4 v[NV];
    float s = 0.f;
#pragma unroll
    for (int i = 0; i < NV; ++i) {
        const int c = (lane + 64 * i) * 4;
        if (c < d) {
            v[i] = *reinterpret_cast<const f32x4*>(xr + c);
            s += v[i][0] + v[i][1] + v[i][2] + v[i][3];
        }
    }
    const float mean = wave_sum(s) / (float)d;
    float q = 0.f;
#pragma unroll
    for (int i = 0; i < NV; ++i) {
        const int c = (lane + 64 * i) * 4;
        if (c < d) {
#pragma unroll
            for (int e = 0; e < 4; ++e) {
                const float t = v[i][e] - mean;
                q += t * t;
            }
        }
    }
    const float var = wave_sum(q) / (float)d;
    const float rstd = 1.0f / sqrtf(var + eps);
    float* yr = y + row * d;
#pragma unroll
    for (int i = 0; i < NV; ++i) {
        const int c = (lane + 64 * i) * 4;
        if (c < d) {
            const f32x4 gm = *reinterpret_cast<const f32x4*>(gamma + c);
            const f32x4 bt = *reinterpret_cast<const f32x4*>(beta + c);
            f32x4 o;
#pragma unroll
            for (int e = 0; e < 4; ++e) {
                float t = (v[i][e] - mean) * rstd * gm[e] + bt[e];
                if (act == AVD_ACT_GELU) t = gelu_erf(t);
                else if (act == AVD_ACT_SILU) t = silu(t);
                else if (act == AVD_ACT_RELU) t = fmaxf(t, 0.f);
                else if (act == AVD_ACT_LEAKY_RELU) t = t > 0.f ? t : 0.1f * t;
                o[e] = t;
            }
            *reinterpret_cast<f32x4*>(yr + c) = o;
        }
    }
}

static int nv_for(int d) { return (d + 255) / 256; }

int rmsnorm_f32(const float* x, RowMap xm, const float* scale, float* y, RowMap ym, int64_t rows, int d, float eps,
                hipStream_t st) {
    AVD_REQUIRE(x && scale && y, AVD_EINVAL, "rmsnorm: null pointer");
    AVD_REQUIRE(rows >= 0 && d > 0, AVD_EINVAL, "rmsnorm: bad dims");
    AVD_REQUIRE(d % 4 == 0 && d <= 256 * ROW_MAXV, AVD_EUNSUPPORTED, "rmsnorm: d=%d must be a multiple of 4, <= %d", d,
                256 * ROW_MAXV);
    AVD_REQUIRE(xm.ld % 4 == 0 && ym.ld % 4 == 0 && aligned16(x) && aligned16(y) && aligned16(scale), AVD_EUNSUPPORTED,
                "rmsnorm: rows must be 16-byte aligned");
    if (rows == 0) return AVD_OK;
    const int tag = prof_tag_id("rmsnorm_kernel<%d>", nv_for(d));
    ProfScope prof(tag, 8.0 * (double)rows * d, st);
    const unsigned grid = (unsigned)((rows + 3) / 4);
    const float isd = (float)sqrt((double)d);
    switch (nv_for(d)) {
#define AVD_CASE(NV) case NV: hipLaunchKernelGGL(rmsnorm_kernel<NV>, dim3(grid), dim3(256), 0, st, x, xm, scale, y, ym, rows, d, eps, isd); break;
        AVD_CASE(1) AVD_CASE(2) AVD_CASE(3) AVD_CASE(4) AVD_CASE(5) AVD_CASE(6) AVD_CASE(7) AVD_CASE(8)
#undef AVD_CASE
    }
    AVD_CHECK_LAUNCH("rmsnorm");
    return AVD_OK;
}

__global__ __launch_bounds__(256) void rowss_kernel(const float* __restrict__ x, float* __restrict__ ss, int64_t rows, int d) {
    const int lane = threadIdx.x & 63;
    const int64_t row = (int64_t)blockIdx.x * 4 + (threadIdx.x >> 6);
    if (row >= rows) return;
    const float* xr = x + row * d;
    float s = 0.f;
    for (int c = lane * 4; c < d; c += 256) {
        const f32x4 v = *reinterpret_cast<const f32x4*>(xr + c);
        s += v[0] * v[0] + v[1] * v[1] + v[2] * v[2] + v[3] * v[3];
    }
    s = wave_sum(s);
    if (lane == 0) ss[row] = s;
}

int rowss_f32(const float* x, float* ss, int64_t rows, int d, hipStream_t st) {
    AVD_REQUIRE(x && ss && rows > 0 && d > 0 && d % 4 == 0 && aligned16(x), AVD_EINVAL, "rowss: bad arguments");
    static const int tag = prof_tag_id("rowss_kernel");
    ProfScope prof(tag, 4.0 * (double)rows * d, st);
    hipLaunchKernelGGL(rowss_kernel, dim3((unsigned)((rows + 3) / 4)), dim3(256), 0, st, x, ss, rows, d);
    AVD_CHECK_LAUNCH("rowss");
    return AVD_OK;
}

__global__ __launch_bounds__(256) void bounds_kernel(const float* __restrict__ x, float* __restrict__ out, int64_t rows, int d) {
    const int lane = threadIdx.x & 63;
    const int64_t row = (int64_t)blockIdx.x * 4 + (threadIdx.x >> 6);
    if (row >= rows) return;
    const float* xr = x + row * d;
    float s = 0.f, m = 0.f;
    bool bad = false;
    for (int c = lane; c < d; c += 64) {
        const float v = xr[c];
        s += v * v;
        m = fmaxf(m, fabsf(v));
        bad = bad || v != v;
    }
    s = wave_sum(s);
#pragma unroll
    for (int o = 32; o > 0; o >>= 1) m = fmaxf(m, __shfl_xor(m, o, 64));
    bad = __any(bad);
    if (lane == 0) {
        const float nrm = bad ? __builtin_nanf("") : sqrtf(s);
        const float mx = bad ? __builtin_nanf("") : m;
        atomicMax(reinterpret_cast<unsigned int*>(out), __float_as_uint(mx));
        atomicMax(reinterpret_cast<unsigned int*>(out) + 1, __float_as_uint(nrm));
    }
}
__global__ void bounds_init_kernel(float* out) { out[threadIdx.x] = 0.f; }

int weight_bounds_f32(const float* x, int64_t rows, int d, float* out2, hipStream_t st) {
    AVD_REQUIRE(x && out2 && rows > 0 && d > 0, AVD_EINVAL, "weight_bounds: bad arguments");
    hipLaunchKernelGGL(bounds_init_kernel, dim3(1), dim3(2), 0, st, out2);
    hipLaunchKernelGGL(bounds_kernel, dim3((unsigned)((rows + 3) / 4)), dim3(256), 0, st, x, out2, rows, d);
    AVD_CHECK_LAUNCH("weight_bounds");
    return AVD_OK;
}

int layernorm_act_f32(const float* x, const float* gamma, const float* beta, float* y, int64_t rows, int d, float eps,
                      int act, hipStream_t st) {
    AVD_REQUIRE(x && gamma && beta && y, AVD_EINVAL, "layernorm: null pointer");
    AVD_REQUIRE(rows >= 0 && d > 0, AVD_EINVAL, "layernorm: bad dims");
    AVD_REQUIRE(d % 4 == 0 && d <= 256 * ROW_MAXV, AVD_EUNSUPPORTED, "layernorm: d=%d must be a multiple of 4, <= %d",
                d, 256 * ROW_MAXV);
    AVD_REQUIRE(aligned16(x) && aligned16(y) && aligned16(gamma) && aligned16(beta), AVD_EUNSUPPORTED,
                "layernorm: pointers must be 16-byte aligned");
    if (rows == 0) return AVD_OK;
    const int tag = prof_tag_id("layernorm_act_kernel<%d>", nv_for(d));
    ProfScope prof(tag, 8.0 * (double)rows * d, st);
    const unsigned grid = (unsigned)((rows + 3) / 4);
    switch (nv_for(d)) {
#define AVD_CASE(NV) case NV: hipLaunchKernelGGL(layernorm_act_kernel<NV>, dim3(grid), dim3(256), 0, st, x, gamma, beta, y, rows, d, eps, act); break;
        AVD_CASE(1) AVD_CASE(2) AVD_CASE(3) AVD_CASE(4) AVD_CASE(5) AVD_CASE(6) AVD_CASE(7) AVD_CASE(8)
#undef AVD_CASE
    }
    AVD_CHECK_LAUNCH("layernorm_act");
    return AVD_OK;
}

}

extern "C" int avd_rmsnorm_f32(const float* x, const float* scale, float* y, int64_t rows, int d, float eps,
                               avd_stream_t stream) {
    return avd::rmsnorm_f32(x, avd::RowMap{d, 0, 0}, scale, y, avd::RowMap{d, 0, 0}, rows, d, eps,
                            static_cast<hipStream_t>(stream));
}

extern "C" int avd_weight_bounds_f32(const float* w, int64_t rows, int cols, float* out2, avd_stream_t stream) {
    return avd::weight_bounds_f32(w, rows, cols, out2, static_cast<hipStream_t>(stream));
}

extern "C" int avd_layernorm_act_f32(const float* x, const float* gamma, const float* beta, float* y, int64_t rows,
                                     int d, float eps, int act, avd_stream_t stream) {
    return avd::layernorm_act_f32(x, gamma, beta, y, rows, d, eps, act, static_cast<hipStream_t>(stream));
}
```

### multimodal_diffusion_amd/csrc/tokens.hip

```cpp
#include "avd_common.h"

#include <stdlib.h>
#include <type_traits>
#include <cmath>
#include <initializer_list>

namespace avd {

__global__ void temb_kernel(const int64_t* __restrict__ t, const float* __restrict__ freqs, float* __restrict__ out,
                            int B, int dim, float neg_log_mp) {
    const int half = dim >> 1;
    const int i = blockIdx.x * blockDim.x + threadIdx.x;
    if (i >= B * dim) return;
    const int b = i / dim, c = i % dim;
    float v = 0.f;
    if (c < 2 * half) {
        const int k = c < half ? c : c - half;
        const float f = freqs ? freqs[k] : expf(neg_log_mp * (float)k / (float)half);
        const float a = (float)t[b] * f;
        v = c < half ? cosf(a) : sinf(a);
    }
    out[i] = v;
}

// ... 2833 lines not shown
                         int canvas_hop, int guide_hop) {
    AVD_REQUIRE(B > 0 && T_train > 0, AVD_EINVAL, "eps_unpatch_ddim: bad dims");
    Tube g;
    if (int rc = make_tube(g, C, T, H, W, t, h, w)) return rc;
    AVD_REQUIRE(aligned16(x0_hist), AVD_EUNSUPPORTED, "eps_unpatch_ddim: x0_hist must be 16-byte aligned");
    const UpdateArgs a{eps1, z, t_now, t_prev, abar, T_train, 0.f, eta, noise, z_out, B};
    UpdateKeys k;
    const CanvasDims cv{C, T, canvas_hop, (int64_t)H * W};
    const CanvasDims gcv{C, T, guide_hop, (int64_t)H * W};
    if (int rc = check_fused_update("eps_unpatch_ddim", a, g.per, key, t_last, x0_hist, guide, nullptr, k, canvas_hop ? &cv : nullptr,
                                    guide_hop ? &gcv : nullptr)) return rc;
    static const int tag = prof_tag_id("eps_unpatch_ddim_kernel");
    ProfScope prof(tag, 12.0 * (double)B * g.per, st);
    with_update_pack(k, true, [&](auto... p) { launch_unpatch(a, g, st, p...); });
    AVD_CHECK_LAUNCH("eps_unpatch_ddim");
    return AVD_OK;
}

template <bool SEEDED, class... Key>
__global__ void cfg_untoken_ddim_audio_kernel(const float* __restrict__ eps2, const float* __restrict__ z,
                                              const int64_t* __restrict__ t_now, const int64_t* __restrict__ t_prev,
                                              const float* __restrict__ abar, int T_train, float guidance, float eta,
                                              const float* __restrict__ noise, float* __restrict__ z_out, int B, int Ca,
                                              int F, int len, int stride, int Na, Key... nk) {
    constexpr bool DPM = PackHas<DpmState, Key...>::value, GUIDED = PackHas<GuideState, Key...>::value;
    constexpr bool CTL = PackHas<CfgState, Key...>::value, COND = PackHas<CondOnly, Key...>::value;
    constexpr bool CANVAS = PackHas<CanvasKey, Key...>::value, CGUIDED = PackHas<CanvasGuideState, Key...>::value;
    static_assert(PackOk<SEEDED, Key...>::value, "not a pack of the fused update kernels (see PackOk)");
    const int64_t i = (int64_t)blockIdx.x * blockDim.x + threadIdx.x;
    if (i >= (int64_t)B * Ca * F) return;
    const int f = (int)(i % F);
    const int c = (int)((i / F) % Ca);
    const int b = (int)(i / ((int64_t)F * Ca));
    const int L = (Na - 1) * stride + len;
    const int D = Ca * len;
    constexpr bool SLOT = PackHas<SlotTimes, Key...>::value;
    [[maybe_unused]] int tb = b;
    if constexpr (SLOT) {
        const int sl = f / len;
        tb = b * Na + (sl > Na - 1 ? Na - 1 : sl);
        if (t_now[tb] == t_prev[tb]) {
            z_out[i] = z[i];
            return;
        }
    }
    [[maybe_unused]] CfgCoef cc{guidance, 0.f, 1.f};
    if constexpr (CTL) cc = cfg_coef(pack_get<CfgState>(nk...), guidance, b);
    constexpr bool SCFG = PackHas<SlotCfgState, Key...>::value;
    [[maybe_unused]] SlotCfgCoef sf{guidance, 0.f, 1.f, 0.f, 0.f, false};
    if constexpr (SCFG) sf = slot_cfg_coef(pack_get<SlotCfgState>(nk...), t_now, T_train, guidance, tb);
    float e = 0.f;
    [[maybe_unused]] bool apg = false;
    if constexpr (CTL) {
        const CfgState cs = pack_get<CfgState>(nk...);
        apg = cs.apg != nullptr;
        if (apg) {
            const float cv = f < L ? ola_gather(eps2 + (int64_t)b * Na * D, D, c, len, stride, Na, f) : 0.f;
            const float uv = f < L ? ola_gather(eps2 + ((int64_t)B + b) * Na * D, D, c, len, stride, Na, f) : 0.f;
            const float dv = apg_dir(apg_d0(cv, uv), cs.apg_beta, cs.apg_mom ? cs.apg_mom[i] : 0.f);
            if (cs.apg_mom) cs.apg_mom[i] = dv;
            e = apg_eps(cv, dv, cs.apg[(int64_t)b * 4 + 2], cs.apg[(int64_t)b * 4 + 1]);
        }
    }
    if constexpr (COND) {
        if (f < L) e = ola_gather(eps2 + (int64_t)b * Na * D, D, c, len, stride, Na, f);
    } else if (!(CTL && apg) && f < L) {
        int n_hi = f / stride;
        if (n_hi > Na - 1) n_hi = Na - 1;
        int n_lo = (f - len + 1 <= 0) ? 0 : (f - len + stride) / stride;
        float acc = 0.f, cnt = 0.f;
        const float* tc = eps2 + (int64_t)b * Na * D;
        const float* tn = eps2 + ((int64_t)B + b) * Na * D;
        for (int n = n_lo; n <= n_hi; ++n) {
            const int64_t o = (int64_t)n * D + c * len + (f - n * stride);
            const float vn = tn[o];
            acc += cfg_combine(tc[o], vn, SCFG ? sf.g : CTL ? cc.g : guidance);
            cnt += 1.f;
        }
        e = acc / fmaxf(cnt, 1e-8f);
        if constexpr (SCFG) {
            if (sf.apg) {
                const float cv = ola_gather(tc, D, c, len, stride, Na, f), uv = ola_gather(tn, D, c, len, stride, Na, f);
                if constexpr (PackHas<SlotMomentum, Key...>::value) {
                    const SlotMomentum sm = pack_get<SlotMomentum>(nk...);
                    const float dv = apg_dir(apg_d0(cv, uv), sm.beta, sm.buf[i]);
                    sm.buf[i] = dv;
                    e = apg_eps(cv, dv, sf.w, sf.k);
                } else e = apg_eps(cv, apg_d0(cv, uv), sf.w, sf.k);
            } else e = cfg_rescale(e, sf.phi, sf.s);
        }
    }
    if constexpr (CTL) e = cfg_rescale(e, cc.phi, cc.s);
    const Ddim cf = ddim_coef(t_now, t_prev, abar, T_train, eta, SLOT ? tb : b);
    auto fin = [&](float v) {
        if constexpr (GUIDED)
            return guide_apply1(pack_get<GuideState>(nk...), guide_coef(abar, T_train, t_prev[b]), b, i, i - (int64_t)b * Ca * F, v);
        else if constexpr (CGUIDED)
            return canvas_guide_apply1(pack_get<CanvasGuideState>(nk...), guide_coef(abar, T_train, t_prev[b]), b, i,
                                       i - (int64_t)b * Ca * F, c, f, 0, 1, v);
        else if constexpr (PackHas<ClipGuideState, Key...>::value)
            return clip_guide_apply1(pack_get<ClipGuideState>(nk...), guide_coef(abar, T_train, t_prev[tb]), b, c, f, 0, 1, v);
        else
            return v;
    };
    [[maybe_unused]] float zn = 0.f;
    if constexpr (PackHas<SlotKey, Key...>::value) {
        zn = slot_normal4(pack_get<SlotKey>(nk...), b, c, f, 0, 1, (uint32_t)t_now[tb])[c & 3];
    } else if constexpr (CANVAS) {
        zn = canvas_normal4(pack_get<CanvasKey>(nk...), b, c, f, 0, 1, (uint32_t)t_now[b])[c & 3];
    } else if constexpr (SEEDED) {
        NoiseKey k;
        if constexpr (GUIDED || CTL || COND || DPM) k = pack_get<NoiseKey>(nk...);
        else k = NoiseKey(nk...);
        const int64_t el = i - (int64_t)b * Ca * F;
        zn = philox_normal4(k, (uint32_t)(el >> 2), k.s0 + (uint32_t)b, (uint32_t)t_now[b])[(int)(el & 3)];
    }
    if constexpr (DPM) {
        const DpmState ds = pack_get<DpmState>(nk...);
        const Dpm d = dpm_coef(ds.t_last, t_now, t_prev, abar, T_train, SEEDED ? eta : 0.f, SLOT ? tb : b);
        const float x = z[i], x0 = ddim_x0(cf, x, e);
        z_out[i] = fin(dpm_apply(d, x, x0, d.c_1 != 0.f ? ds.x0_hist[i] : 0.f, zn, SEEDED));
        ds.x0_hist[i] = x0;
    } else if constexpr (SEEDED) {
        z_out[i] = fin(ddim_apply(cf, z[i], e, zn));
    } else {
        z_out[i] = fin(ddim_apply(cf, z[i], e, eta > 0.f ? noise[i] : 0.f));
    }
}

template <class... P>
static void launch_untoken(const UpdateArgs& a, const AudioGeom& ag, hipStream_t st, P... p) {
    constexpr bool SEEDED = PackHas<NoiseKey, P...>::value || PackHas<CanvasKey, P...>::value || PackHas<SlotKey, P...>::value;
    const int64_t n = (int64_t)a.B * ag.Ca * ag.F;
    hipLaunchKernelGGL((cfg_untoken_ddim_audio_kernel<SEEDED, P...>), dim3((unsigned)((n + 255) / 256)), dim3(256), 0, st, a.eps, a.z,
                       a.t_now, a.t_prev, a.abar, a.T_train, a.guidance, a.eta, a.noise, a.z_out, a.B, ag.Ca, ag.F, ag.len, ag.stride,
                       ag.Na, p...);
}

int cfg_untoken_ddim_audio_f32(const float* eps2, const float* z, const int64_t* t_now, const int64_t* t_prev,
                               const float* abar, int T_train, float guidance, float eta, const float* noise,
                               float* z_out, int B, int Ca, int F, int len, int stride, hipStream_t st, const avd_noise_key* key,
                               const int64_t* t_last, float* x0_hist, const avd_latent_guide* guide, const avd_cfg_control* ctl,
                               int canvas_hop, int guide_hop, int slots, const avd_apg_control* apg, const avd_slot_key* skey = nullptr,
                               const avd_clip_guide* cguide = nullptr, const avd_slot_cfg* scfg = nullptr) {
    AVD_REQUIRE(B > 0 && Ca > 0 && T_train > 0, AVD_EINVAL, "cfg_untoken_ddim_audio: bad dims");
    AVD_REQUIRE(len > 0 && stride > 0 && F >= len, AVD_EUNSUPPORTED, "cfg_untoken_ddim_audio: bad chunking");
    AVD_REQUIRE(!slots || stride == len, AVD_EUNSUPPORTED,
                "cfg_untoken_ddim_audio: slot timesteps need non-overlapping chunks (stride %d == len %d)", stride, len);
    const UpdateArgs a{eps2, z, t_now, t_prev, abar, T_train, guidance, eta, noise, z_out, B};
    const int64_t per = (int64_t)Ca * F;
    UpdateKeys k;
    const CanvasDims cv{Ca, F, canvas_hop, 1};
    const CanvasDims gcv{Ca, F, guide_hop, 1};
    const AudioGeom ag{Ca, F, len, stride, audio_na(F, len, stride)};
    SlotCfgState sc{};
    SlotMomentum sm{};
    const SlotGeom sg{ag.Na, (int64_t)Ca * len, (int64_t)Ca * len, 0};
    if (scfg) {
        AVD_REQUIRE(slots > 0, AVD_EINVAL, "cfg_untoken_ddim_audio: a slot CFG control rides with slot timesteps (slots > 0)");
        if (int rc = make_slot_cfg(scfg, B, sg.S, sg.per_slot, per, {z, z_out, x0_hist}, eps2, (int64_t)2 * B * ag.Na * Ca * len * 4, sc,
                                   sm)) return rc;
    }
    if (int rc = check_fused_update("cfg_untoken_ddim_audio", a, per, key, t_last, x0_hist, guide, ctl, k, canvas_hop ? &cv : nullptr,
                                    guide_hop ? &gcv : nullptr, apg, (int64_t)2 * B * ag.Na * Ca * len * 4, skey)) return rc;
    if (int rc = check_slot_update("cfg_untoken_ddim_audio", a, slots, ag.Na, key, guide, ctl, canvas_hop, guide_hop, k, skey,
                                   SlotKeyDims{Ca, len, 1}, cguide, F)) return rc;
    k.scfg = scfg != nullptr;
    k.sc = sc;
    k.smom = sm.buf != nullptr;
    k.sm = sm;
    if (scfg && sc.mode != SLOT_CFG_TABLE) {
        const int64_t half = (int64_t)ag.Na * Ca * len;
        if (int rc = run_slot_cfg_stats<CFG_SRC_AUDIO>(scfg, sc, eps2, eps2 + B * half, half, t_now, t_prev, guidance, T_train, B, sg, Tube{},
                                                       st, SlotMomentumAt{sm.buf, sm.beta, per, len, F})) return rc;
    }
    if (apg) {
        const int64_t half = (int64_t)ag.Na * Ca * len;
        if (int rc = run_apg_stats<CFG_SRC_AUDIO>(apg, ctl ? ctl->guidance : nullptr, guidance, eps2, eps2 + B * half, half, B, per,
                                                  Tube{}, ag, st)) return rc;
    }
    if (ctl && ctl->rescale) {
        const int64_t half = (int64_t)ag.Na * Ca * len;
        if (int rc = run_cfg_stats<CFG_SRC_AUDIO>(ctl, eps2, eps2 + B * half, half, guidance, B, per, ag, st)) return rc;
    }
    with_update_pack(k, false, [&](auto... p) { launch_untoken(a, ag, st, p...); });
    AVD_CHECK_LAUNCH("cfg_untoken_ddim_audio");
    return AVD_OK;
}

int eps_untoken_ddim_audio_f32(const float* eps1, const float* z, const int64_t* t_now, const int64_t* t_prev, const float* abar,
                               int T_train, float eta, const float* noise, float* z_out, int B, int Ca, int F, int len, int stride,
                               hipStream_t st, const avd_noise_key* key, const int64_t* t_last, float* x0_hist,
                               const avd_latent_guide* guide, int canvas_hop, int guide_hop) {
    AVD_REQUIRE(B > 0 && Ca > 0 && T_train > 0, AVD_EINVAL, "eps_untoken_ddim_audio: bad dims");
    AVD_REQUIRE(len > 0 && stride > 0 && F >= len, AVD_EUNSUPPORTED, "eps_untoken_ddim_audio: bad chunking");
    const UpdateArgs a{eps1, z, t_now, t_prev, abar, T_train, 0.f, eta, noise, z_out, B};
    UpdateKeys k;
    const CanvasDims cv{Ca, F, canvas_hop, 1};
    const CanvasDims gcv{Ca, F, guide_hop, 1};
    if (int rc = check_fused_update("eps_untoken_ddim_audio", a, (int64_t)Ca * F, key, t_last, x0_hist, guide, nullptr, k,
                                    canvas_hop ? &cv : nullptr, guide_hop ? &gcv : nullptr)) return rc;
    const AudioGeom ag{Ca, F, len, stride, audio_na(F, len, stride)};
    with_update_pack(k, true, [&](auto... p) { launch_untoken(a, ag, st, p...); });
    AVD_CHECK_LAUNCH("eps_untoken_ddim_audio");
    return AVD_OK;
}

__global__ __launch_bounds__(256) void assemble_kernel(float* __restrict__ X2, const float* __restrict__ temb,
                                                       const float* __restrict__ Xp, int B, int N, int d, int tdim,
                                                       int Nt, int Np, int target_first, int64_t total4) {
    const int64_t i = (int64_t)blockIdx.x * 256 + threadIdx.x;
    if (i >= total4) return;
    const int d4 = d >> 2;
    const int col = (int)(i % d4) * 4;
    const int64_t row = i / d4;
    const int n = (int)(row % N);
    const int bb = (int)(row / N);
    const int half = bb >= B, b = half ? bb - B : bb;
    const int t0 = target_first ? 0 : Np;
    const bool is_t = n >= t0 && n < t0 + Nt;
    f32x4 v;
    if (is_t) {
        if (col >= d - tdim) {
            v = *reinterpret_cast<const f32x4*>(temb + (int64_t)b * tdim + (col - (d - tdim)));
        } else {
            if (!half) return;
            v = *reinterpret_cast<const f32x4*>(X2 + ((int64_t)b * N + n) * d + col);
        }
    } else {
        const int np = target_first ? n - Nt : n;
        v = half ? f32x4{0.f, 0.f, 0.f, 0.f} : *reinterpret_cast<const f32x4*>(Xp + ((int64_t)b * Np + np) * d + col);
    }
    *reinterpret_cast<f32x4*>(X2 + row * d + col) = v;
}

int assemble_f32(float* X2, const float* temb, const float* Xp, int B, int N, int d, int tdim, int Nt, int Np,
                 int target_first, hipStream_t st) {
    const int64_t total4 = (int64_t)2 * B * N * (d >> 2);
    static const int tag = prof_tag_id("assemble_kernel");
    ProfScope prof(tag, 4.0 * (2.0 * B * N * d + (double)B * Nt * (d - tdim) + (double)B * Np * d), st);
    hipLaunchKernelGGL(assemble_kernel, dim3((unsigned)((total4 + 255) / 256)), dim3(256), 0, st, X2, temb, Xp, B, N, d,
                       tdim, Nt, Np, target_first, total4);
    AVD_CHECK_LAUNCH("assemble");
    return AVD_OK;
}

struct SlotMap {
    int S, tok;
};
template <class... Slot>
__global__ __launch_bounds__(256) void assemble_rows_kernel(float* __restrict__ X2, const int64_t* __restrict__ t_now,
                                                            const float* __restrict__ freqs, const float* __restrict__ Xp,
                                                            float* __restrict__ ss, int B, int N, int d, int tdim, int Nt, int Np,
                                                            int target_first, float neg_log_mp, RowSegs seg, Slot... sl) {
    const int lane = threadIdx.x & 63;
    const int64_t row = (int64_t)blockIdx.x * 4 + (threadIdx.x >> 6);
    if (row >= seg.rows()) return;
    int n, bb;
    seg.locate(row, bb, n);
    const int half = bb >= B, b = half ? bb - B : bb;
    const int t0 = target_first ? 0 : Np;
    const bool is_t = n >= t0 && n < t0 + Nt;
    const int da = d - tdim, th = tdim >> 1;
    float tf = 0.f;
    if constexpr (sizeof...(Slot) != 0) {
        const SlotMap sm = SlotMap(sl...);
        if (is_t) tf = (float)t_now[b * sm.S + (n - t0) / sm.tok];
    } else {
        tf = is_t ? (float)t_now[b] : 0.f;
    }
    float acc = 0.f;
    for (int col = lane * 4; col < d; col += 256) {
        f32x4 v;
        bool store = true;
        if (is_t) {
            if (col >= da) {
#pragma unroll
                for (int e = 0; e < 4; ++e) {
                    const int c = col - da + e;
                    float x = 0.f;
                    if (c < 2 * th) {
                        const int k = c < th ? c : c - th;
                        const float f = freqs ? freqs[k] : expf(neg_log_mp * (float)k / (float)th);
                        const float a = tf * f;
                        x = c < th ? cosf(a) : sinf(a);
                    }
                    v[e] = x;
                }
            } else {
                v = *reinterpret_cast<const f32x4*>(X2 + ((int64_t)b * N + n) * d + col);
                store = half != 0;
            }
        } else {
            const int np = target_first ? n - Nt : n;
            v = half ? f32x4{0.f, 0.f, 0.f, 0.f} : *reinterpret_cast<const f32x4*>(Xp + ((int64_t)b * Np + np) * d + col);
        }
        if (store) *reinterpret_cast<f32x4*>(X2 + row * d + col) = v;
        acc += v[0] * v[0] + v[1] * v[1] + v[2] * v[2] + v[3] * v[3];
    }
    acc = wave_sum(acc);
    if (ss && lane == 0) ss[row] = acc;
}

int assemble_rows_f32(float* X2, const int64_t* t_now, const float* freqs, const float* Xp, float* ss, int B, int N, int d, int tdim,
                      int Nt, int Np, int target_first, float max_period, hipStream_t st, const RowSegs* short_null, int slots,
                      int slot_tok) {
    AVD_REQUIRE(!slots || (slot_tok > 0 && (int64_t)slots * slot_tok == Nt), AVD_EINVAL,
                "assemble_rows: %d slots of %d tokens are not the %d target rows", slots, slot_tok, Nt);
    AVD_REQUIRE(!short_null || (target_first && Np >= 1 && short_null->samples[0] == B && short_null->samples[1] == B && short_null->tok[0] == N &&
                                short_null->tok[1] == Nt + 1 && short_null->m0 == (int64_t)B * N), AVD_EINVAL,
                "assemble_rows: a short null half is B samples of N rows, then B of the target rows and one prompt row behind them");
    const RowSegs seg = short_null ? *short_null : RowSegs::uniform(2 * B, N);
    const int64_t rows = seg.rows();
    static const int tag = prof_tag_id("assemble_rows_kernel");
    ProfScope prof(tag, 4.0 * ((double)rows * d + (double)B * Nt * (d - tdim) + (double)B * Np * d), st);
    if (slots)
        hipLaunchKernelGGL(assemble_rows_kernel<SlotMap>, dim3((unsigned)((rows + 3) / 4)), dim3(256), 0, st, X2, t_now, freqs, Xp, ss, B, N,
                           d, tdim, Nt, Np, target_first, -(float)log((double)max_period), seg, SlotMap{slots, slot_tok});
    else
        hipLaunchKernelGGL(assemble_rows_kernel<>, dim3((unsigned)((rows + 3) / 4)), dim3(256), 0, st, X2, t_now, freqs, Xp, ss, B, N, d, tdim,
                           Nt, Np, target_first, -(float)log((double)max_period), seg);
    AVD_CHECK_LAUNCH("assemble_rows");
    return AVD_OK;
}

__global__ __launch_bounds__(256) void qkv3_replicate_kernel(unsigned char* __restrict__ img, int Bt, int H, int Npad, int first_sample,
                                                             int n_samples, int src, int n_keys) {
    const int dup = n_keys - 1 - src;
    const int64_t i = (int64_t)blockIdx.x * 256 + threadIdx.x;
    const int64_t total = (int64_t)2 * n_samples * H * dup * 24;
    if (i >= total) return;
    const int c = (int)(i % 8), plane = (int)(i / 8 % 3);
    int64_t r = i / 24;
    const int j = (int)(r % dup);
    r /= dup;
    const int h = (int)(r % H);
    r /= H;
    const int b = (int)(r % n_samples), part = 1 + (int)(r / n_samples);
    unsigned char* base = img + (((int64_t)part * Bt + first_sample + b) * H + h) * (int64_t)Npad * QKV3_ROWB;
    const int dst = src + 1 + j;
    const u32x4 v = *reinterpret_cast<const u32x4*>(base + (int64_t)src * QKV3_ROWB + plane * 128 + ((c ^ qkv3_swizzle(part, src)) << 4));
    *reinterpret_cast<u32x4*>(base + (int64_t)dst * QKV3_ROWB + plane * 128 + ((c ^ qkv3_swizzle(part, dst)) << 4)) = v;
}

int qkv3_replicate(void* img, int img_samples, int H, int n_keys, int first_sample, int n_samples, int src, hipStream_t st) {
    AVD_REQUIRE(img && aligned16(img), AVD_EINVAL, "qkv3_replicate: null or misaligned image");
    AVD_REQUIRE(H > 0 && n_keys > 0 && src >= 0 && src < n_keys && first_sample >= 0 && n_samples > 0 && first_sample + n_samples <= img_samples,
                AVD_EINVAL, "qkv3_replicate: bad geometry (samples %d + %d of %d, token %d of %d keys)", first_sample, n_samples, img_samples,
                src, n_keys);
    const int dup = n_keys - 1 - src;
    if (dup == 0) return AVD_OK;
    const int64_t total = (int64_t)2 * n_samples * H * dup * 24;
    AVD_REQUIRE((total + 255) / 256 < (1ll << 31), AVD_EUNSUPPORTED, "qkv3_replicate: grid too large");
    static const int tag = prof_tag_id("qkv3_replicate_kernel");
    ProfScope prof(tag, 32.0 * (double)total, st);
    hipLaunchKernelGGL(qkv3_replicate_kernel, dim3((unsigned)((total + 255) / 256)), dim3(256), 0, st, static_cast<unsigned char*>(img),
                       img_samples, H, qkv3_npad(n_keys), first_sample, n_samples, src, n_keys);
    AVD_CHECK_LAUNCH("qkv3_replicate");
    return AVD_OK;
}

__global__ __launch_bounds__(256) void assemble_cond_kernel(float* __restrict__ X1, const float* __restrict__ temb,
                                                            const float* __restrict__ Xp, int B, int N, int d, int tdim, int Nt,
                                                            int Np, int target_first, int64_t total4) {
    const int64_t i = (int64_t)blockIdx.x * 256 + threadIdx.x;
    if (i >= total4) return;
    const int d4 = d >> 2;
    const int col = (int)(i % d4) * 4;
    const int64_t row = i / d4;
    const int n = (int)(row % N);
    const int b = (int)(row / N);
    const int t0 = target_first ? 0 : Np;
    const bool is_t = n >= t0 && n < t0 + Nt;
    f32x4 v;
    if (is_t) {
        if (col < d - tdim) return;
        v = *reinterpret_cast<const f32x4*>(temb + (int64_t)b * tdim + (col - (d - tdim)));
    } else {
        const int np = target_first ? n - Nt : n;
        v = *reinterpret_cast<const f32x4*>(Xp + ((int64_t)b * Np + np) * d + col);
    }
    *reinterpret_cast<f32x4*>(X1 + row * d + col) = v;
}

int assemble_cond_f32(float* X1, const float* temb, const float* Xp, int B, int N, int d, int tdim, int Nt, int Np, int target_first,
                      hipStream_t st) {
    const int64_t total4 = (int64_t)B * N * (d >> 2);
    static const int tag = prof_tag_id("assemble_cond_kernel");
    ProfScope prof(tag, 4.0 * 2.0 * ((double)B * Nt * tdim + (double)B * Np * d), st);
    hipLaunchKernelGGL(assemble_cond_kernel, dim3((unsigned)((total4 + 255) / 256)), dim3(256), 0, st, X1, temb, Xp, B, N, d, tdim, Nt, Np,
                       target_first, total4);
    AVD_CHECK_LAUNCH("assemble_cond");
    return AVD_OK;
}

__global__ __launch_bounds__(256) void assemble_rows_cond_kernel(float* __restrict__ X1, const int64_t* __restrict__ t_now,
                                                                 const float* __restrict__ freqs, const float* __restrict__ Xp,
                                                                 float* __restrict__ ss, int B, int N, int d, int tdim, int Nt, int Np,
                                                                 int target_first, float neg_log_mp) {
    const int lane = threadIdx.x & 63;
    const int64_t row = (int64_t)blockIdx.x * 4 + (threadIdx.x >> 6);
    if (row >= (int64_t)B * N) return;
    const int n = (int)(row % N);
    const int b = (int)(row / N);
    const int t0 = target_first ? 0 : Np;
    const bool is_t = n >= t0 && n < t0 + Nt;
    const int da = d - tdim, th = tdim >> 1;
    const float tf = is_t ? (float)t_now[b] : 0.f;
    float acc = 0.f;
    for (int col = lane * 4; col < d; col += 256) {
        f32x4 v;
        bool store = true;
        if (is_t) {
            if (col >= da) {
#pragma unroll
                for (int e = 0; e < 4; ++e) {
                    const int c = col - da + e;
                    float x = 0.f;
                    if (c < 2 * th) {
                        const int k = c < th ? c : c - th;
                        const float f = freqs ? freqs[k] : expf(neg_log_mp * (float)k / (float)th);
                        const float a = tf * f;
                        x = c < th ? cosf(a) : sinf(a);
                    }
                    v[e] = x;
                }
            } else {
                v = *reinterpret_cast<const f32x4*>(X1 + row * d + col);
                store = false;
            }
        } else {
            const int np = target_first ? n - Nt : n;
            v = *reinterpret_cast<const f32x4*>(Xp + ((int64_t)b * Np + np) * d + col);
        }
        if (store) *reinterpret_cast<f32x4*>(X1 + row * d + col) = v;
        acc += v[0] * v[0] + v[1] * v[1] + v[2] * v[2] + v[3] * v[3];
    }
    acc = wave_sum(acc);
    if (ss && lane == 0) ss[row] = acc;
}

int assemble_rows_cond_f32(float* X1, const int64_t* t_now, const float* freqs, const float* Xp, float* ss, int B, int N, int d,
                           int tdim, int Nt, int Np, int target_first, float max_period, hipStream_t st) {
    const int64_t rows = (int64_t)B * N;
    static const int tag = prof_tag_id("assemble_rows_cond_kernel");
    ProfScope prof(tag, 4.0 * ((double)B * N * d + (double)B * Np * d), st);
    hipLaunchKernelGGL(assemble_rows_cond_kernel, dim3((unsigned)((rows + 3) / 4)), dim3(256), 0, st, X1, t_now, freqs, Xp, ss, B, N, d,
                       tdim, Nt, Np, target_first, -(float)log((double)max_period));
    AVD_CHECK_LAUNCH("assemble_rows_cond");
    return AVD_OK;
}

__global__ void sched_advance_kernel(const int64_t* __restrict__ sched, int n_sched, int32_t* cursor,
                                     int64_t* __restrict__ t_now, int64_t* __restrict__ t_prev, int B) {
    __shared__ int cur;
    if (threadIdx.x == 0) cur = *cursor;
    __syncthreads();
    int i = cur;
    if (i < 0) i = 0;
    if (i > n_sched - 2) i = n_sched - 2;
    const int64_t a = sched[i], p = sched[i + 1];
    for (int b = threadIdx.x; b < B; b += blockDim.x) {
        t_now[b] = a;
        t_prev[b] = p;
    }
    __syncthreads();
    if (threadIdx.x == 0) *cursor = cur + 1;
}

__global__ void sched_advance_ms_kernel(const int64_t* __restrict__ sched, int n_sched, int32_t* cursor, int64_t* __restrict__ t_last,
                                        int64_t* __restrict__ t_now, int64_t* __restrict__ t_prev, int B) {
    __shared__ int cur;
    if (threadIdx.x == 0) cur = *cursor;
    __syncthreads();
    int i = cur;
    if (i < 0) i = 0;
    if (i > n_sched - 2) i = n_sched - 2;
    const int64_t a = sched[i], p = sched[i + 1];
    const int64_t l = i > 0 && sched[i - 1] > a ? sched[i - 1] : -1;
    for (int b = threadIdx.x; b < B; b += blockDim.x) {
        t_last[b] = l;
        t_now[b] = a;
        t_prev[b] = p;
    }
    __syncthreads();
    if (threadIdx.x == 0) *cursor = cur + 1;
}

}

using namespace avd;

extern "C" int avd_timestep_embedding_f32(const int64_t* t, const float* freqs, float* out, int B, int dim,
                                          float max_period, avd_stream_t stream) {
    return temb_f32(t, freqs, out, B, dim, max_period, static_cast<hipStream_t>(stream));
}
extern "C" int avd_tube_patch_f32(const float* z, float* tok, int B, int C, int T, int H, int W, int t, int h, int w,
                                  avd_stream_t stream) {
    AVD_REQUIRE(aligned16(z) && aligned16(tok), AVD_EUNSUPPORTED, "tube_patch: pointers must be 16-byte aligned");
    return tube_patch_f32(z, tok, B, C, T, H, W, t, h, w, static_cast<hipStream_t>(stream));
}
extern "C" int avd_tube_unpatch_f32(const float* tok, float* z, int B, int C, int T, int H, int W, int t, int h, int w,
                                    avd_stream_t stream) {
    AVD_REQUIRE(aligned16(z) && aligned16(tok), AVD_EUNSUPPORTED, "tube_unpatch: pointers must be 16-byte aligned");
    return tube_unpatch_f32(tok, z, B, C, T, H, W, t, h, w, static_cast<hipStream_t>(stream));
}
extern "C" int avd_audio_tokens_f32(const float* z, float* tok, int B, int Ca, int F, int len, int stride,
                                    avd_stream_t stream) {
    return audio_tokens_f32(z, tok, B, Ca, F, len, stride, static_cast<hipStream_t>(stream));
}
extern "C" int avd_audio_untokens_f32(const float* tok, const float* window, float* z, int B, int Ca, int F, int len, int stride,
                                      avd_stream_t stream) {
    return audio_untokens_f32(tok, window, z, B, Ca, F, len, stride, static_cast<hipStream_t>(stream));
}
extern "C" int avd_ddim_step_f32(const float* x_t, const float* eps_hat, const int64_t* t_now, const int64_t* t_prev,
                                 const float* alpha_bar, int T_train, float eta, const float* noise, float* x_prev,
                                 int B, int64_t per_sample, avd_stream_t stream) {
    return ddim_step_f32(x_t, eps_hat, t_now, t_prev, alpha_bar, T_train, eta, noise, x_prev, B, per_sample,
                         static_cast<hipStream_t>(stream));
}
extern "C" int avd_cfg_unpatch_ddim_f32(const float* eps2, const float* z, const int64_t* t_now, const int64_t* t_prev,
                                        const float* alpha_bar, int T_train, float guidance, float eta,
                                        const float* noise, float* z_out, int B, int C, int T, int H, int W, int t,
                                        int h, int w, avd_stream_t stream) {
    AVD_REQUIRE(aligned16(eps2) && aligned16(z) && aligned16(z_out) && (!noise || aligned16(noise)), AVD_EUNSUPPORTED,
                "cfg_unpatch_ddim: pointers must be 16-byte aligned");
    return cfg_unpatch_ddim_f32(eps2, z, t_now, t_prev, alpha_bar, T_train, guidance, eta, noise, z_out, B, C, T, H, W, t,
                                h, w, static_cast<hipStream_t>(stream), nullptr, nullptr, nullptr, nullptr, nullptr, 0, 0, 0, nullptr);
}
extern "C" int avd_cfg_unpatch_ddim_slots_f32(const float* eps2, const float* z, const int64_t* t_now, const int64_t* t_prev,
                                              const float* alpha_bar, int T_train, float guidance, int slots, float* z_out, int B, int C,
                                              int T, int H, int W, int t, int h, int w, avd_stream_t stream) {
    AVD_REQUIRE(aligned16(eps2) && aligned16(z) && aligned16(z_out), AVD_EUNSUPPORTED,
                "cfg_unpatch_ddim_slots: pointers must be 16-byte aligned");
    AVD_REQUIRE(slots > 0, AVD_EINVAL, "cfg_unpatch_ddim_slots: slots must be > 0 (got %d)", slots);
    return cfg_unpatch_ddim_f32(eps2, z, t_now, t_prev, alpha_bar, T_train, guidance, 0.f, nullptr, z_out, B, C, T, H, W, t, h, w,
                                static_cast<hipStream_t>(stream), nullptr, nullptr, nullptr, nullptr, nullptr, 0, 0, slots, nullptr);
}
extern "C" int avd_cfg_untoken_ddim_audio_slots_f32(const float* eps2, const float* z, const int64_t* t_now, const int64_t* t_prev,
                                                    const float* alpha_bar, int T_train, float guidance, int slots, float* z_out, int B,
                                                    int Ca, int F, int len, int stride, avd_stream_t stream) {
    AVD_REQUIRE(slots > 0, AVD_EINVAL, "cfg_untoken_ddim_audio_slots: slots must be > 0 (got %d)", slots);
    return cfg_untoken_ddim_audio_f32(eps2, z, t_now, t_prev, alpha_bar, T_train, guidance, 0.f, nullptr, z_out, B, Ca, F, len, stride,
                                      static_cast<hipStream_t>(stream), nullptr, nullptr, nullptr, nullptr, nullptr, 0, 0, slots, nullptr);
}
extern "C" int avd_fifo_shift_f32(const avd_noise_key* key, int64_t t, int64_t c, const float* z_in, float* z_out, float* popped, int B,
                                  int64_t outer, int slots, int slot_len, int64_t inner, avd_stream_t stream) {
    return fifo_shift_f32(key, t, c, z_in, z_out, popped, B, outer, slots, slot_len, inner, static_cast<hipStream_t>(stream));
}
extern "C" int avd_cfg_unpatch_dpmpp_2m_slots_f32(const float* eps2, const float* z, const int64_t* t_last, const int64_t* t_now,
                                                  const int64_t* t_prev, const float* alpha_bar, int T_train, float guidance, int slots,
                                                  float* x0_hist, float* z_out, int B, int C, int T, int H, int W, int t, int h, int w,
                                                  avd_stream_t stream) {
    AVD_REQUIRE(aligned16(eps2) && aligned16(z) && aligned16(z_out), AVD_EUNSUPPORTED,
                "cfg_unpatch_dpmpp_2m_slots: pointers must be 16-byte aligned");
    AVD_REQUIRE(slots > 0, AVD_EINVAL, "cfg_unpatch_dpmpp_2m_slots: slots must be > 0 (got %d)", slots);
    AVD_REQUIRE(t_last && x0_hist, AVD_EINVAL, "cfg_unpatch_dpmpp_2m_slots: null t_last or x0_hist");
    return cfg_unpatch_ddim_f32(eps2, z, t_now, t_prev, alpha_bar, T_train, guidance, 0.f, nullptr, z_out, B, C, T, H, W, t, h, w,
                                static_cast<hipStream_t>(stream), nullptr, t_last, x0_hist, nullptr, nullptr, 0, 0, slots, nullptr);
}
extern "C" int avd_cfg_untoken_dpmpp_2m_audio_slots_f32(const float* eps2, const float* z, const int64_t* t_last, const int64_t* t_now,
                                                        const int64_t* t_prev, const float* alpha_bar, int T_train, float guidance,
                                                        int slots, float* x0_hist, float* z_out, int B, int Ca, int F, int len, int stride,
                                                        avd_stream_t stream) {
    AVD_REQUIRE(slots > 0, AVD_EINVAL, "cfg_untoken_dpmpp_2m_audio_slots: slots must be > 0 (got %d)", slots);
    AVD_REQUIRE(t_last && x0_hist, AVD_EINVAL, "cfg_untoken_dpmpp_2m_audio_slots: null t_last or x0_hist");
    return cfg_untoken_ddim_audio_f32(eps2, z, t_now, t_prev, alpha_bar, T_train, guidance, 0.f, nullptr, z_out, B, Ca, F, len, stride,
                                      static_cast<hipStream_t>(stream), nullptr, t_last, x0_hist, nullptr, nullptr, 0, 0, slots, nullptr);
}
extern "C" int avd_cfg_unpatch_ddim_slots_seeded_f32(const float* eps2, const float* z, const int64_t* t_last, const int64_t* t_now,
                                                     const int64_t* t_prev, const float* alpha_bar, int T_train, float guidance, float eta,
                                                     const avd_slot_key* key, int slots, float* x0_hist, float* z_out, int B, int C, int T,
                                                     int H, int W, int t, int h, int w, avd_stream_t stream) {
    AVD_REQUIRE(aligned16(eps2) && aligned16(z) && aligned16(z_out), AVD_EUNSUPPORTED,
                "cfg_unpatch_ddim_slots_seeded: pointers must be 16-byte aligned");
    AVD_REQUIRE(slots > 0, AVD_EINVAL, "cfg_unpatch_ddim_slots_seeded: slots must be > 0 (got %d)", slots);
    AVD_REQUIRE(key, AVD_EINVAL, "cfg_unpatch_ddim_slots_seeded: null slot key");
    return cfg_unpatch_ddim_f32(eps2, z, t_now, t_prev, alpha_bar, T_train, guidance, eta, nullptr, z_out, B, C, T, H, W, t, h, w,
                                static_cast<hipStream_t>(stream), nullptr, t_last, x0_hist, nullptr, nullptr, 0, 0, slots, nullptr, key);
}
extern "C" int avd_cfg_untoken_ddim_audio_slots_seeded_f32(const float* eps2, const float* z, const int64_t* t_last, const int64_t* t_now,
                                                           const int64_t* t_prev, const float* alpha_bar, int T_train, float guidance,
                                                           float eta, const avd_slot_key* key, int slots, float* x0_hist, float* z_out,
                                                           int B, int Ca, int F, int len, int stride, avd_stream_t stream) {
    AVD_REQUIRE(slots > 0, AVD_EINVAL, "cfg_untoken_ddim_audio_slots_seeded: slots must be > 0 (got %d)", slots);
    AVD_REQUIRE(key, AVD_EINVAL, "cfg_untoken_ddim_audio_slots_seeded: null slot key");
    return cfg_untoken_ddim_audio_f32(eps2, z, t_now, t_prev, alpha_bar, T_train, guidance, eta, nullptr, z_out, B, Ca, F, len, stride,
                                      static_cast<hipStream_t>(stream), nullptr, t_last, x0_hist, nullptr, nullptr, 0, 0, slots, nullptr, key);
}
extern "C" int avd_cfg_unpatch_ddim_slots_guided_f32(const float* eps2, const float* z, const int64_t* t_last, const int64_t* t_now,
                                                     const int64_t* t_prev, const float* alpha_bar, int T_train, float guidance, float eta,
                                                     const avd_slot_key* key, const avd_clip_guide* guide, int slots, float* x0_hist,
                                                     float* z_out, int B, int C, int T, int H, int W, int t, int h, int w,
                                                     avd_stream_t stream) {
    AVD_REQUIRE(aligned16(eps2) && aligned16(z) && aligned16(z_out), AVD_EUNSUPPORTED,
                "cfg_unpatch_ddim_slots_guided: pointers must be 16-byte aligned");
    AVD_REQUIRE(slots > 0, AVD_EINVAL, "cfg_unpatch_ddim_slots_guided: slots must be > 0 (got %d)", slots);
    AVD_REQUIRE(guide, AVD_EINVAL, "cfg_unpatch_ddim_slots_guided: null clip guide");
    AVD_REQUIRE(key || !(eta > 0.f), AVD_EINVAL, "cfg_unpatch_ddim_slots_guided: eta > 0 needs a slot key");
    return cfg_unpatch_ddim_f32(eps2, z, t_now, t_prev, alpha_bar, T_train, guidance, eta, nullptr, z_out, B, C, T, H, W, t, h, w,
                                static_cast<hipStream_t>(stream), nullptr, t_last, x0_hist, nullptr, nullptr, 0, 0, slots, nullptr, key, guide);
}
extern "C" int avd_cfg_untoken_ddim_audio_slots_guided_f32(const float* eps2, const float* z, const int64_t* t_last, const int64_t* t_now,
                                                           const int64_t* t_prev, const float* alpha_bar, int T_train, float guidance,
                                                           float eta, const avd_slot_key* key, const avd_clip_guide* guide, int slots,
                                                           float* x0_hist, float* z_out, int B, int Ca, int F, int len, int stride,
                                                           avd_stream_t stream) {
    AVD_REQUIRE(slots > 0, AVD_EINVAL, "cfg_untoken_ddim_audio_slots_guided: slots must be > 0 (got %d)", slots);
    AVD_REQUIRE(guide, AVD_EINVAL, "cfg_untoken_ddim_audio_slots_guided: null clip guide");
    AVD_REQUIRE(key || !(eta > 0.f), AVD_EINVAL, "cfg_untoken_ddim_audio_slots_guided: eta > 0 needs a slot key");
    return cfg_untoken_ddim_audio_f32(eps2, z, t_now, t_prev, alpha_bar, T_train, guidance, eta, nullptr, z_out, B, Ca, F, len, stride,
                                      static_cast<hipStream_t>(stream), nullptr, t_last, x0_hist, nullptr, nullptr, 0, 0, slots, nullptr, key,
                                      guide);
}
extern "C" int avd_cfg_unpatch_ddim_slots_cfg_f32(const float* eps2, const float* z, const int64_t* t_last, const int64_t* t_now,
                                                  const int64_t* t_prev, const float* alpha_bar, int T_train, float guidance, float eta,
// ... 270 lines not shown
```

Measured before the change: 125.1 steps/s.

## Fuse split3 images into assemble and final rmsnorm, skipping separate split passes

The token-assembly kernel now also writes the bf16x3 split image and per-64-column sum-of-squares straight into the carved core workspace. This lets the core skip its first split3_rows pass. The final RMSNorm of the trimmed last block likewise writes the head's input split image directly, including zero padding rows, so the head skips its own split3 pass. Each change removes a full read/write of the activations and one kernel launch per CFG half, at the cost of workspace-layout coupling between embed, core and head, which is checked at runtime.

```diff
diff --git a/multimodal_diffusion_amd/csrc/avd_common.h b/multimodal_diffusion_amd/csrc/avd_common.h
--- a/multimodal_diffusion_amd/csrc/avd_common.h
+++ b/multimodal_diffusion_amd/csrc/avd_common.h
@@ -90,6 +90,12 @@
     __host__ __device__ __forceinline__ int64_t row(int sample, int token) const {
         return sample < samples[0] ? (int64_t)sample * tok[0] + token : m0 + (int64_t)(sample - samples[0]) * tok[1] + token;
     }
+};
+
+struct RowImages {
+    unsigned char* img[2];
+    float* ss[2];
+    int64_t first[2], rows[2], pad[2];
 };
 
 struct TubeGather {
@@ -248,6 +254,8 @@
 int split3_f32(const float* x, int64_t ld, void* out, int64_t rows, int K, hipStream_t st, float h2_scale = 0.f);
 int split3_rows_f32(const float* x, RowMap xm, void* out, int64_t rows, int K, hipStream_t st, float h2_scale = 0.f, float* ss = nullptr);
 int rmsnorm_split3_f32(const float* x, const float* scale, void* out, int64_t rows, int d, float eps, hipStream_t st, float h2_scale = 0.f);
+int rmsnorm_image_f32(const float* x, RowMap xm, const float* scale, void* img, int64_t img_row0, int64_t rows, int64_t zero_rows,
+                      int d, float eps, hipStream_t st);
 int layernorm_act_split3_f32(const float* x, const float* gamma, const float* beta, void* out, int64_t rows, int d, float eps, int act,
                              hipStream_t st, float h2_scale = 0.f);
 bool gemm_bf16x3_supported(int64_t M, int N, int K);
diff --git a/multimodal_diffusion_amd/csrc/composite.hip b/multimodal_diffusion_amd/csrc/composite.hip
--- a/multimodal_diffusion_amd/csrc/composite.hip
+++ b/multimodal_diffusion_amd/csrc/composite.hip
@@ -73,7 +73,7 @@
                  int target_first, hipStream_t st);
 int assemble_rows_f32(float* X2, const int64_t* t_now, const float* freqs, const float* Xp, float* ss, int B, int N, int d, int tdim,
                       int Nt, int Np, int target_first, float max_period, hipStream_t st, const RowSegs* short_null = nullptr, int slots = 0,
-                      int slot_tok = 0);
+                      int slot_tok = 0, const RowImages* images = nullptr);
 int qkv3_replicate(void* img, int img_samples, int H, int n_keys, int first_sample, int n_samples, int src, hipStream_t st);
 int cfg_unpatch_ddim_f32(const float* eps2, const float* z, const int64_t* t_now, const int64_t* t_prev,
                          const float* abar, int T_train, float guidance, float eta, const float* noise, float* z_out,
@@ -187,6 +187,9 @@
 static int g_core_trim = 1;
 static int64_t core_trim_floats(const avd_core_weights* w, int B, int N) { return (int64_t)B * N * w->d; }
 static int g_cfg_offset = 0;
+static int g_tail_image = 1;
+static int g_front_image = 1;
+struct CoreTail { void* img; int64_t zero_rows; };
 
 static int g_cfg_dedup = 1;
 [[maybe_unused]] static const bool g_cfg_dedup_env_applied = [] {
@@ -248,10 +251,20 @@
            !g_mlp_fused && gemm_bf16x3_resmap_supported(terms) && core_use_split(w, (int64_t)B2 * N) && core_use_split_fold(w);
 }
 
+struct CoreFirst { void* hx; float* ss; };
+static CoreFirst core_first_image(const avd_core_weights* w, int B, int N, void* ws, int64_t ws_bytes) {
+    const int64_t M = (int64_t)B * N;
+    Carver cs{static_cast<char*>(ws), 0, ws_bytes};
+    cs.take((core_split_wide_bytes(w, B, N) + 3) / 4);
+    cs.take((split3_bytes(M, w->d) + 3) / 4);
+    cs.take(((w->attn_mode == 1 ? attn_fp8_ws_bytes(B, N, w->n_heads) : 0) + 3) / 4);
+    void* hx = cs.take((split3_bytes(M, w->d) + 3) / 4);
+    return CoreFirst{hx, cs.take(M * (w->d / 64))};
+}
 static int core_forward(const avd_core_weights* w, const float* x, float* y, int B, int N, int out_row0,
                         int n_out_rows, const unsigned char* kpm, void* ws, int64_t ws_bytes, hipStream_t st,
                         const float* ss_first = nullptr, const RowSegs* segs = nullptr, int plan_samples = 0,
-                        hipEvent_t lead = nullptr, int lead_after = 0) {
+                        hipEvent_t lead = nullptr, int lead_after = 0, const CoreTail* tail = nullptr, const CoreFirst* first = nullptr) {
     if (int rc = check_core(w)) return rc;
     AVD_REQUIRE(x && y && B > 0 && N > 0, AVD_EINVAL, "core: bad input");
     AVD_REQUIRE(out_row0 >= 0 && n_out_rows > 0 && out_row0 + n_out_rows <= N, AVD_EINVAL, "core: bad output row window");
@@ -276,6 +289,8 @@
     AVD_REQUIRE(!(w->attn_mode == 1 && !core_use_split(w, M)), AVD_EUNSUPPORTED,
                 "core: attn_mode 1 (fp8 attention) reads the q|k|v image of the split-operand projections, which these weights / shapes "
                 "do not take (every block needs its *_weight3 images; 3 d, d and mlp_hidden must be multiples of 256, d of 16)");
+    AVD_REQUIRE(!(tail || first) || (!kpm && core_use_split(w, M) && core_use_split_fold(w)), AVD_EUNSUPPORTED,
+                "core: an output tail or a first image needs the folded split path");
     if (!kpm && core_use_split(w, M)) {
         const int terms = w->split_terms;
         Carver cs{static_cast<char*>(ws), 0, ws_bytes};
@@ -295,6 +310,7 @@
             float* yc = cs.take(core_trim_floats(w, B, N));
             const bool fused = g_mlp_fused && !ns && mlp_bf16x3_supported(d, hid, terms) && gemm_bf16x3_resmap_supported(terms);
             AVD_REQUIRE(cs.ok, AVD_EWORKSPACE, "core: workspace carve %lld > %lld bytes", (long long)cs.used, (long long)cs.cap);
+            AVD_REQUIRE(!tail || (trim && tail->img), AVD_EUNSUPPORTED, "core: an output tail needs the trimmed last block");
             const RowSegs seg = segs ? *segs : RowSegs::uniform(B, N);
             const int64_t Mr = seg.rows();
             const float qscale = scale * 1.4426950408889634f;
@@ -307,7 +323,9 @@
                 if (lead && l == 0 && n == lead_after) AVD_HIP(hipEventRecord(lead, st));
                 return (int)AVD_OK;
             };
-            if (int rc = split3_rows_f32(cur, rd, hx, Mr, d, st, 0.f, ss)) return rc;
+            AVD_REQUIRE(!first || (first->hx == hx && first->ss == ss), AVD_EINVAL, "core: the first image is not where this call carves it");
+            if (!first)
+                if (int rc = split3_rows_f32(cur, rd, hx, Mr, d, st, 0.f, ss)) return rc;
             for (int l = 0; l < w->n_layers; ++l) {
                 const avd_block_weights& b = w->blocks[l];
                 const bool last = l == w->n_layers - 1;
@@ -335,6 +353,7 @@
                                                      nullptr, 0.f, nullptr, nullptr, 0, nullptr, Mcp)) return rc;
                         }
                     }
+                    if (tail) return rmsnorm_image_f32(yc, rd, w->final_norm_scale, tail->img, 0, Mc, tail->zero_rows, d, w->norm_eps, st);
                     return rmsnorm_f32(yc, rd, w->final_norm_scale, y, segs ? rd : RowMap{d, nq, (int64_t)N * d}, Mc, d, w->norm_eps, st);
                 }
                 if (int rc = in_proj(b)) return rc;
@@ -486,9 +505,12 @@
     return split_path > fp32_path ? split_path : fp32_path;
 }
 
+static bool head_takes_image(const avd_head_weights* w, int64_t rows) { return w->split_terms != 3 && head_use_split(w, rows); }
+static void* head_input_image(void* ws) { return ws; }
+
 static int head_forward(const avd_head_weights* w, const float* h, RowMap hm, int64_t rows, float* out, void* ws,
-                        int64_t ws_bytes, hipStream_t st, int64_t plan_rows = 0) {
-    AVD_REQUIRE(w && h && out, AVD_EINVAL, "head: null pointer");
+                        int64_t ws_bytes, hipStream_t st, int64_t plan_rows = 0, bool have_img = false) {
+    AVD_REQUIRE(w && (h || have_img) && out, AVD_EINVAL, "head: null pointer");
     AVD_REQUIRE(w->d_in > 0 && w->hidden > 0 && w->d_out > 0 && w->n_shared >= 0, AVD_EINVAL, "head: bad dims");
     AVD_REQUIRE(w->input_proj_weight && w->out_proj_weight, AVD_EINVAL, "head: null weights");
     AVD_REQUIRE(w->n_shared == 0 || (w->shared_lin_weight && w->shared_lin_bias && w->shared_ln_weight && w->shared_ln_bias),
@@ -511,7 +533,8 @@
         void* imgA = cv.take((split3_bytes(rows, wide) + 3) / 4);
         void* imgB = cv.take((split3_bytes(rows, wide) + 3) / 4);
         float* t2 = cv.take(rows * w->hidden);
-        if (int rc = split3_rows_f32(h, hm, imgA, rows, w->d_in, st, asc(0))) return rc;
+        if (!have_img)
+            if (int rc = split3_rows_f32(h, hm, imgA, rows, w->d_in, st, asc(0))) return rc;
         if (int rc = gemm_bf16x3(imgA, w->input_proj_weight3, w->input_proj_bias, nullptr, nullptr, imgB, rows, w->hidden, w->d_in, AVD_ACT_NONE,
                                  terms, st, h2 ? asc(0) * wsc(0) : 1.f, h2 ? asc(1) : 1.f, nullptr, 0.f, nullptr, nullptr, 0, nullptr, plan_rows)) return rc;
         void* cur = imgB;
@@ -526,6 +549,7 @@
         return gemm_bf16x3(cur, w->out_proj_weight3, w->out_proj_bias, nullptr, out, nullptr, rows, w->d_out, w->hidden, AVD_ACT_NONE, terms, st,
                            h2 ? asc(1 + n) * wsc(1 + n) : 1.f, 1.f, nullptr, 0.f, nullptr, nullptr, 0, nullptr, plan_rows);
     }
+    AVD_REQUIRE(!have_img, AVD_EUNSUPPORTED, "head: an input image needs the split-operand mode");
     float* t1 = cv.take(rows * w->hidden);
     float* t2 = cv.take(rows * w->hidden);
     if (int rc = gemm_f32(h, hm, w->input_proj_weight, w->input_proj_bias, nullptr, rh, t1, rh, rows, w->hidden, w->d_in, AVD_ACT_NONE, st)) return rc;
@@ -576,7 +600,7 @@
 
 static int embed_cfg_pair(const avd_embed_desc* e, const float* z, const float* Wt, const float* bt,
                           const int64_t* t_now, const float* Xp, float* tok_ws, float* X2, hipStream_t st, float* ss_out = nullptr,
-                          bool cond_only = false, const RowSegs* short_null = nullptr, int slots = 0) {
+                          bool cond_only = false, const RowSegs* short_null = nullptr, int slots = 0, const RowImages* images = nullptr) {
     if (int rc = check_embed(e)) return rc;
     int slot_tok = 0;
     if (slots) {
@@ -588,6 +612,7 @@
     AVD_REQUIRE(z && Wt && t_now && tok_ws && X2 && (e->Np == 0 || Xp), AVD_EINVAL, "embed: null pointer");
     AVD_REQUIRE(!short_null || (!cond_only && !e->temb_add && e->target_first && e->Np >= 1), AVD_EINVAL,
                 "embed: the short null half is the concat-mode CFG pair with the target rows first");
+    AVD_REQUIRE(!images || short_null, AVD_EINVAL, "embed: row images go with the short null half");
     const int B = e->B, d = e->d, N = e->Nt + e->Np, D = embed_tok_dim(e);
     float* tok = tok_ws;
     float* temb = tok_ws + align_up((int64_t)B * e->Nt * D * 4) / 4;
@@ -617,7 +642,7 @@
     if (cond_only)
         return assemble_rows_cond_f32(X2, t_now, e->temb_freqs, Xp, ss_out, B, N, d, e->tdim, e->Nt, e->Np, e->target_first, 10000.f, st);
     return assemble_rows_f32(X2, t_now, e->temb_freqs, Xp, ss_out, B, N, d, e->tdim, e->Nt, e->Np, e->target_first, 10000.f, st,
-                             short_null, slots, slot_tok);
+                             short_null, slots, slot_tok, images);
 }
 
 struct AuxState { hipStream_t aux = nullptr; hipEvent_t fork = nullptr, join = nullptr, lead = nullptr; };
@@ -718,6 +743,8 @@
     {"attn_m16", "AVD_ATTN_M16", &g_attn_m16, INT_MIN, INT_MAX, false},
     {"core_trim", "AVD_CORE_TRIM", &g_core_trim, INT_MIN, INT_MAX, true},
     {"cfg_offset", "AVD_CFG_OFFSET", &g_cfg_offset, 0, 3, false},
+    {"tail_image", "AVD_TAIL_IMAGE", &g_tail_image, 0, 1, false},
+    {"front_image", "AVD_FRONT_IMAGE", &g_front_image, 0, 1, false},
     {"mlp_fused", "AVD_MLP_FUSED", &g_mlp_fused, INT_MIN, INT_MAX, false},
     {"gemm_tile", "AVD_GEMM_TILE", &g_gemm_force_tile, INT_MIN, INT_MAX, false},
     {"gemm_stages", "AVD_GEMM_STAGES", &g_gemm_stages, INT_MIN, INT_MAX, false},
@@ -832,12 +859,26 @@
                        core_dedup_ok(s->core, 2 * e.B, p.N, e.Nt);
     const bool two = s->split_streams == 2 ? dedup : s->split_streams != 0;
     const RowSegs seg{(int64_t)e.B * p.N, {p.N, e.Nt + 1}, {e.B, e.B}};
-    if (int rc = embed_cfg_pair(&e, z, s->adapt_w, s->adapt_b, t_now, Xp, tok, X2, st, ssx, false, dedup ? &seg : nullptr, slots)) return rc;
+    const bool front = dedup && g_front_image;
+    const int64_t hc = p.core / 2;
+    const CoreFirst f_c = core_first_image(s->core, two ? e.B : 2 * e.B, p.N, core_ws, two ? hc : p.core);
+    const CoreFirst f_n = core_first_image(s->core, e.B, p.N, static_cast<char*>(core_ws) + hc, hc);
+    auto pad256 = [](int64_t rows) { return (rows + 255) / 256 * 256 - rows; };
+    const int64_t rows_n = seg.rows() - seg.m0;
+    const RowImages one_img{{static_cast<unsigned char*>(f_c.hx), nullptr}, {f_c.ss, nullptr}, {0, 0}, {seg.rows(), 0}, {pad256(seg.rows()), 0}};
+    const RowImages two_img{{static_cast<unsigned char*>(f_c.hx), static_cast<unsigned char*>(f_n.hx)}, {f_c.ss, f_n.ss}, {0, seg.m0},
+                            {seg.m0, rows_n}, {pad256(seg.m0), pad256(rows_n)}};
+    if (int rc = embed_cfg_pair(&e, z, s->adapt_w, s->adapt_b, t_now, Xp, tok, X2, st, ssx, false, dedup ? &seg : nullptr, slots,
+                                front ? (two ? &two_img : &one_img) : nullptr)) return rc;
     const int row0 = e.target_first ? 0 : e.Np;
     const RowMap hm{e.d, e.Nt, (int64_t)p.N * e.d};
+    const bool img_rows = g_tail_image && (p.rows / 2) % 128 == 0;
     if (dedup && !two) {
-        if (int rc = core_forward(s->core, X2, X2, 2 * e.B, p.N, 0, e.Nt, nullptr, core_ws, p.core, st, nullptr, &seg)) return rc;
-        if (int rc = head_forward(s->head, X2, RowMap{e.d, 0, 0}, p.rows, eps2, head_ws, p.head, st)) return rc;
+        const bool img = img_rows && head_takes_image(s->head, p.rows);
+        const CoreTail tl{head_input_image(head_ws), 0};
+        if (int rc = core_forward(s->core, X2, X2, 2 * e.B, p.N, 0, e.Nt, nullptr, core_ws, p.core, st, nullptr, &seg, 0, nullptr, 0,
+                                  img ? &tl : nullptr, front ? &f_c : nullptr)) return rc;
+        if (int rc = head_forward(s->head, X2, RowMap{e.d, 0, 0}, p.rows, eps2, head_ws, p.head, st, 0, img)) return rc;
     } else if (!two) {
         if (int rc = core_forward(s->core, X2, X2, 2 * e.B, p.N, row0, e.Nt, nullptr, core_ws, p.core, st, have_ss ? ssx : nullptr)) return rc;
         if (int rc = head_forward(s->head, X2 + (int64_t)row0 * e.d, hm, p.rows, eps2, head_ws, p.head, st)) return rc;
@@ -847,7 +888,7 @@
         hipStream_t g_aux = ax.aux;
         hipEvent_t g_fork = ax.fork, g_join = ax.join;
         const int64_t half_rows = (int64_t)e.B * p.N * e.d;
-        const int64_t hc = p.core / 2, hh = p.head / 2;
+        const int64_t hh = p.head / 2;
         AVD_HIP(hipEventRecord(g_fork, st));
         AVD_HIP(hipStreamWaitEvent(g_aux, g_fork, 0));
         struct TwoStreams {
@@ -858,14 +899,18 @@
             const RowSegs null_seg{0, {p.N, e.Nt + 1}, {0, e.B}};
             float* xn = X2 + seg.m0 * e.d;
             float* eps_n = eps2 + (p.rows / 2) * p.D;
+            const int64_t hr = p.rows / 2;
+            const bool img = img_rows && head_takes_image(s->head, hr);
+            char* head_n = static_cast<char*>(head_ws) + hh;
+            const int64_t pad = (hr + 255) / 256 * 256 - hr;
+            const CoreTail tl_c{head_input_image(head_ws), pad}, tl_n{head_input_image(head_n), pad};
             if (int rc = core_forward(s->core, X2, X2, e.B, p.N, 0, e.Nt, nullptr, core_ws, hc, st, nullptr, nullptr, 2 * e.B,
-                                      g_cfg_offset ? ax.lead : nullptr, g_cfg_offset)) return rc;
-            if (int rc = head_forward(s->head, X2, hm, p.rows / 2, eps2, head_ws, hh, st, p.rows)) return rc;
+                                      g_cfg_offset ? ax.lead : nullptr, g_cfg_offset, img ? &tl_c : nullptr, front ? &f_c : nullptr)) return rc;
+            if (int rc = head_forward(s->head, X2, hm, hr, eps2, head_ws, hh, st, p.rows, img)) return rc;
             if (g_cfg_offset) AVD_HIP(hipStreamWaitEvent(g_aux, ax.lead, 0));
             if (int rc = core_forward(s->core, xn, xn, e.B, p.N, 0, e.Nt, nullptr, static_cast<char*>(core_ws) + hc, hc, g_aux, nullptr,
-                                      &null_seg, 2 * e.B)) return rc;
-            if (int rc = head_forward(s->head, xn, RowMap{e.d, 0, 0}, p.rows / 2, eps_n, static_cast<char*>(head_ws) + hh, hh,
-                                      g_aux, p.rows)) return rc;
+                                      &null_seg, 2 * e.B, nullptr, 0, img ? &tl_n : nullptr, front ? &f_n : nullptr)) return rc;
+            if (int rc = head_forward(s->head, xn, RowMap{e.d, 0, 0}, hr, eps_n, head_n, hh, g_aux, p.rows, img)) return rc;
         }
         for (int half = 0; half < 2 && !dedup; ++half) {
             hipStream_t hs = half ? g_aux : st;
diff --git a/multimodal_diffusion_amd/csrc/rowops.hip b/multimodal_diffusion_amd/csrc/rowops.hip
--- a/multimodal_diffusion_amd/csrc/rowops.hip
+++ b/multimodal_diffusion_amd/csrc/rowops.hip
@@ -32,6 +32,48 @@
             const f32x4 s = *reinterpret_cast<const f32x4*>(scale + c);
             f32x4 o = {s[0] * v[i][0] / den, s[1] * v[i][1] / den, s[2] * v[i][2] / den, s[3] * v[i][3] / den};
             *reinterpret_cast<f32x4*>(yr + c) = o;
+        }
+    }
+}
+
+template <int NV>
+__global__ __launch_bounds__(256) void rmsnorm_image_kernel(const float* __restrict__ x, RowMap xm, const float* __restrict__ scale,
+                                                            unsigned char* __restrict__ img, int64_t img_row0, int64_t rows,
+                                                            int64_t zero_rows, int d, float eps, float sqrt_d) {
+    const int lane = threadIdx.x & 63;
+    const int64_t row = (int64_t)blockIdx.x * 4 + (threadIdx.x >> 6);
+    if (row >= rows + zero_rows) return;
+    const bool live = row < rows;
+    const float* xr = x + (live ? xm.off(row) : 0);
+    f32x4 v[NV];
+    float ss = 0.f;
+#pragma unroll
+    for (int i = 0; i < NV; ++i) {
+        const int c = (lane + 64 * i) * 4;
+        v[i] = f32x4{0.f, 0.f, 0.f, 0.f};
+        if (c < d && live) {
+            v[i] = *reinterpret_cast<const f32x4*>(xr + c);
+            ss += v[i][0] * v[i][0] + v[i][1] * v[i][1] + v[i][2] * v[i][2] + v[i][3] * v[i][3];
+        }
+    }
+    ss = wave_sum(ss);
+    const float den = sqrtf(ss) / sqrt_d + eps;
+#pragma unroll
+    for (int i = 0; i < NV; ++i) {
+        const int c = (lane + 64 * i) * 4;
+        f32x4 o = {0.f, 0.f, 0.f, 0.f};
+        if (c < d && live) {
+            const f32x4 s = *reinterpret_cast<const f32x4*>(scale + c);
+            o = f32x4{s[0] * v[i][0] / den, s[1] * v[i][1] / den, s[2] * v[i][2] / den, s[3] * v[i][3] / den};
+        }
+        f32x4 p;
+#pragma unroll
+        for (int e = 0; e < 4; ++e) p[e] = __shfl_xor(o[e], 1, 64);
+        if (c < d && (lane & 1) == (i & 1)) {
+            const bool lo = !(lane & 1);
+            const f32x4 a = lo ? o : p, b = lo ? p : o;
+            const float w[8] = {a[0], a[1], a[2], a[3], b[0], b[1], b[2], b[3]};
+            store_split8(img, img_row0 + row, c & ~7, d, w);
         }
     }
 }
@@ -116,6 +158,28 @@
     return AVD_OK;
 }
 
+int rmsnorm_image_f32(const float* x, RowMap xm, const float* scale, void* img, int64_t img_row0, int64_t rows, int64_t zero_rows,
+                      int d, float eps, hipStream_t st) {
+    AVD_REQUIRE(x && scale && img, AVD_EINVAL, "rmsnorm_image: null pointer");
+    AVD_REQUIRE(rows >= 0 && zero_rows >= 0 && img_row0 >= 0 && d > 0, AVD_EINVAL, "rmsnorm_image: bad dims");
+    AVD_REQUIRE(d % 16 == 0 && d <= 256 * ROW_MAXV, AVD_EUNSUPPORTED, "rmsnorm_image: d=%d must be a multiple of 16, <= %d", d, 256 * ROW_MAXV);
+    AVD_REQUIRE(xm.ld % 4 == 0 && aligned16(x) && aligned16(scale) && aligned16(img), AVD_EUNSUPPORTED,
+                "rmsnorm_image: rows must be 16-byte aligned");
+    if (rows + zero_rows == 0) return AVD_OK;
+    const int tag = prof_tag_id("rmsnorm_image_kernel<%d>", nv_for(d));
+    ProfScope prof(tag, 4.0 * (double)rows * d + 6.0 * (double)(rows + zero_rows) * d, st);
+    const unsigned grid = (unsigned)((rows + zero_rows + 3) / 4);
+    const float isd = (float)sqrt((double)d);
+    unsigned char* o = static_cast<unsigned char*>(img);
+    switch (nv_for(d)) {
+#define AVD_CASE(NV) case NV: hipLaunchKernelGGL(rmsnorm_image_kernel<NV>, dim3(grid), dim3(256), 0, st, x, xm, scale, o, img_row0, rows, zero_rows, d, eps, isd); break;
+        AVD_CASE(1) AVD_CASE(2) AVD_CASE(3) AVD_CASE(4) AVD_CASE(5) AVD_CASE(6) AVD_CASE(7) AVD_CASE(8)
+#undef AVD_CASE
+    }
+    AVD_CHECK_LAUNCH("rmsnorm_image");
+    return AVD_OK;
+}
+
 __global__ __launch_bounds__(256) void rowss_kernel(const float* __restrict__ x, float* __restrict__ ss, int64_t rows, int d) {
     const int lane = threadIdx.x & 63;
     const int64_t row = (int64_t)blockIdx.x * 4 + (threadIdx.x >> 6);
diff --git a/multimodal_diffusion_amd/csrc/tokens.hip b/multimodal_diffusion_amd/csrc/tokens.hip
--- a/multimodal_diffusion_amd/csrc/tokens.hip
+++ b/multimodal_diffusion_amd/csrc/tokens.hip
@@ -3159,9 +3159,83 @@
     if (ss && lane == 0) ss[row] = acc;
 }
 
+template <class... Slot>
+__global__ __launch_bounds__(256) void assemble_rows_image_kernel(float* __restrict__ X2, const int64_t* __restrict__ t_now,
+                                                                  const float* __restrict__ freqs, const float* __restrict__ Xp, int B,
+                                                                  int N, int d, int tdim, int Nt, int Np, int target_first,
+                                                                  float neg_log_mp, RowSegs seg, RowImages im, Slot... sl) {
+    const int lane = threadIdx.x & 63;
+    const int64_t row = (int64_t)blockIdx.x * 4 + (threadIdx.x >> 6);
+    const int64_t total = seg.rows();
+    if (row >= total + im.pad[0] + im.pad[1]) return;
+    if (row >= total) {
+        const int k = row - total >= im.pad[0];
+        const int64_t r = im.rows[k] + (row - total) - (k ? im.pad[0] : 0);
+        const float zero[8] = {0.f, 0.f, 0.f, 0.f, 0.f, 0.f, 0.f, 0.f};
+        for (int col = lane * 8; col < d; col += 512) store_split8(im.img[k], r, col, d, zero);
+        return;
+    }
+    int n, bb;
+    seg.locate(row, bb, n);
+    const int half = bb >= B, b = half ? bb - B : bb;
+    const int t0 = target_first ? 0 : Np;
+    const bool is_t = n >= t0 && n < t0 + Nt;
+    const int da = d - tdim, th = tdim >> 1;
+    float tf = 0.f;
+    if constexpr (sizeof...(Slot) != 0) {
+        const SlotMap sm = SlotMap(sl...);
+        if (is_t) tf = (float)t_now[b * sm.S + (n - t0) / sm.tok];
+    } else {
+        tf = is_t ? (float)t_now[b] : 0.f;
+    }
+    const int k = im.rows[1] > 0 && row >= im.first[1];
+    const int64_t r = row - im.first[k];
+    for (int col8 = lane * 8; col8 < d; col8 += 512) {
+        float w[8];
+#pragma unroll
+        for (int q = 0; q < 2; ++q) {
+            const int col = col8 + 4 * q;
+            f32x4 v;
+            bool store = true;
+            if (is_t) {
+                if (col >= da) {
+#pragma unroll
+                    for (int e = 0; e < 4; ++e) {
+                        const int c = col - da + e;
+                        float x = 0.f;
+                        if (c < 2 * th) {
+                            const int kf = c < th ? c : c - th;
+                            const float f = freqs ? freqs[kf] : expf(neg_log_mp * (float)kf / (float)th);
+                            const float a = tf * f;
+                            x = c < th ? cosf(a) : sinf(a);
+                        }
+                        v[e] = x;
+                    }
+                } else {
+                    v = *reinterpret_cast<const f32x4*>(X2 + ((int64_t)b * N + n) * d + col);
+                    store = half != 0;
+                }
+            } else {
+                const int np = target_first ? n - Nt : n;
+                v = half ? f32x4{0.f, 0.f, 0.f, 0.f} : *reinterpret_cast<const f32x4*>(Xp + ((int64_t)b * Np + np) * d + col);
+            }
+            if (store) *reinterpret_cast<f32x4*>(X2 + row * d + col) = v;
+#pragma unroll
+            for (int e = 0; e < 4; ++e) w[4 * q + e] = v[e];
+        }
+        store_split8(im.img[k], r, col8, d, w);
+        auto pair = [&](int i) { return __fmaf_rn(w[i], w[i], __fmul_rn(w[i + 1], w[i + 1])); };
+        float s = __fadd_rn(__fadd_rn(pair(0), pair(2)), __fadd_rn(pair(4), pair(6)));
+        s += __shfl_xor(s, 1, 64);
+        s += __shfl_xor(s, 2, 64);
+        s += __shfl_xor(s, 4, 64);
+        if ((lane & 7) == 0) im.ss[k][r * (d >> 6) + (col8 >> 6)] = s;
+    }
+}
+
 int assemble_rows_f32(float* X2, const int64_t* t_now, const float* freqs, const float* Xp, float* ss, int B, int N, int d, int tdim,
                       int Nt, int Np, int target_first, float max_period, hipStream_t st, const RowSegs* short_null, int slots,
-                      int slot_tok) {
+                      int slot_tok, const RowImages* images) {
     AVD_REQUIRE(!slots || (slot_tok > 0 && (int64_t)slots * slot_tok == Nt), AVD_EINVAL,
                 "assemble_rows: %d slots of %d tokens are not the %d target rows", slots, slot_tok, Nt);
     AVD_REQUIRE(!short_null || (target_first && Np >= 1 && short_null->samples[0] == B && short_null->samples[1] == B && short_null->tok[0] == N &&
@@ -3169,6 +3243,24 @@
                 "assemble_rows: a short null half is B samples of N rows, then B of the target rows and one prompt row behind them");
     const RowSegs seg = short_null ? *short_null : RowSegs::uniform(2 * B, N);
     const int64_t rows = seg.rows();
+    if (images) {
+        const RowImages& im = *images;
+        AVD_REQUIRE(im.img[0] && im.ss[0] && aligned16(im.img[0]) && (im.rows[1] == 0 || (im.img[1] && im.ss[1] && aligned16(im.img[1]))) &&
+                    im.first[0] == 0 && im.rows[0] > 0 && im.rows[1] >= 0 && (im.rows[1] == 0 || im.first[1] == im.rows[0]) &&
+                    im.rows[0] + im.rows[1] == rows && im.pad[0] >= 0 && im.pad[1] >= 0 && d % 64 == 0, AVD_EINVAL,
+                    "assemble_rows: the row images must cover the %lld rows once, d %% 64 == 0 (d=%d)", (long long)rows, d);
+        static const int tag_img = prof_tag_id("assemble_rows_image_kernel");
+        const int64_t waves = rows + im.pad[0] + im.pad[1];
+        ProfScope prof(tag_img, 4.0 * ((double)rows * d + (double)B * Nt * (d - tdim) + (double)B * Np * d) + 6.0 * (double)waves * d, st);
+        if (slots)
+            hipLaunchKernelGGL(assemble_rows_image_kernel<SlotMap>, dim3((unsigned)((waves + 3) / 4)), dim3(256), 0, st, X2, t_now, freqs, Xp, B,
+                               N, d, tdim, Nt, Np, target_first, -(float)log((double)max_period), seg, im, SlotMap{slots, slot_tok});
+        else
+            hipLaunchKernelGGL(assemble_rows_image_kernel<>, dim3((unsigned)((waves + 3) / 4)), dim3(256), 0, st, X2, t_now, freqs, Xp, B, N, d,
+                               tdim, Nt, Np, target_first, -(float)log((double)max_period), seg, im);
+        AVD_CHECK_LAUNCH("assemble_rows_image");
+        return AVD_OK;
+    }
     static const int tag = prof_tag_id("assemble_rows_kernel");
     ProfScope prof(tag, 4.0 * ((double)rows * d + (double)B * Nt * (d - tdim) + (double)B * Np * d), st);
     if (slots)
```

New measurement: 125.6 steps/s (median of 6 runs). Within noise of the previous version (+0.4%).
